# voidful/DeSTA2.5-Audio

Hardware: AMD Instinct MI355X
Metric: train steps/sec (node) Whisper-v3+Llama3.1-8B Q-Former6L at 1/2/4/8 MI355X (higher is better)
Workload: dtype bf16

## Files before the change

### desta2.5-audio_amd/csrc/attention.hip

```cpp
#include "common.h"
#include <mutex>
#include "desta_hip.h"

#ifndef ATTN_ABL
#define ATTN_ABL 0
#endif

namespace {

typedef __attribute__((ext_vector_type(4))) __bf16 bf16x4;

struct AttnArgs {
    const bf16_t* Q; const bf16_t* K; const bf16_t* V; bf16_t* O;
    const bf16_t* dO; bf16_t* dQ; bf16_t* dK; bf16_t* dV;
    float* lse; const float* delta;
    float* O32;
    const float* rope_cs;
    long q_bs, q_rs, k_bs, k_rs, v_bs, v_rs, o_bs, o_rs;
    long do_bs, do_rs, dq_bs, dq_rs, dk_bs, dk_rs, dv_bs, dv_rs;
    int B, Hq, Hkv, Sq, Sk;
    int causal;
    const int* kv_start;
    float scale_log2;
    float scale;
// ... 8 lines not shown
}

template <int N> struct stage_vec;
template <> struct stage_vec<1> { typedef __attribute__((ext_vector_type(4))) unsigned type; };
template <> struct stage_vec<2> { typedef __attribute__((ext_vector_type(8))) unsigned type; };
template <> struct stage_vec<4> { typedef __attribute__((ext_vector_type(16))) unsigned type; };
template <int D, int ROWS, int NT = 256> using stage_t = typename stage_vec<ROWS * (D / 8) / NT>::type;

template <int D, int ROWS, int NT = 256>
__device__ __forceinline__ stage_t<D, ROWS, NT> tile_load(const bf16_t* base, long rs, int row0, int max_row) {
    constexpr int CH = D / 8, N = ROWS * CH / NT;
    stage_t<D, ROWS, NT> out;
#pragma unroll
    for (int i = 0; i < N; ++i) {
        const int id = i * NT + threadIdx.x;
        const int r = id / CH, c = id % CH;
        const int gr = min(row0 + r, max_row);
        const uint4 v = *(const uint4*)(base + (long)gr * rs + c * 8);
        out[4 * i + 0] = v.x; out[4 * i + 1] = v.y; out[4 * i + 2] = v.z; out[4 * i + 3] = v.w;
    }
    return out;
}
template <int D, int ROWS, int NT = 256>
__device__ __forceinline__ void tile_store(char* img, const stage_t<D, ROWS, NT>& regs) {
    constexpr int CH = D / 8, N = ROWS * CH / NT;
#pragma unroll
    for (int i = 0; i < N; ++i) {
        const int id = i * NT + threadIdx.x;
        const int r = id / CH, c = id % CH;
        *(uint4*)(img + img_off<D>(r, c)) = make_uint4(regs[4 * i + 0], regs[4 * i + 1], regs[4 * i + 2], regs[4 * i + 3]);
    }
}

template <int D>
__device__ __forceinline__ bf16x8 frag_rows(const char* img, int row0, int ks, int lane) {
    const int r = row0 + (lane & 31);
    return *(const bf16x8*)(img + img_off<D>(r, 2 * ks + (lane >> 5)));
}

template <int D>
__device__ __forceinline__ bf16x8 frag_tr(const char* img, int row0, int col0, int lane) {
    const int i = lane & 15, g = (lane >> 4) & 1, h = lane >> 5;
    const int q = i >> 2, pp = i & 3;
    const int c = col0 + 16 * g + 4 * pp;
    const int r_lo = row0 + 4 * h + q;
    const int a0 = img_off<D>(r_lo, c >> 3) + ((c & 4) << 1);
    const int a1 = img_off<D>(r_lo + 8, c >> 3) + ((c & 4) << 1);
    const bf16x4 lo = __builtin_amdgcn_ds_read_tr16_b64_v4bf16((__attribute__((address_space(3))) bf16x4*)(img + a0));
    const bf16x4 hi = __builtin_amdgcn_ds_read_tr16_b64_v4bf16((__attribute__((address_space(3))) bf16x4*)(img + a1));
    bf16x8 out;
    out[0] = lo[0]; out[1] = lo[1]; out[2] = lo[2]; out[3] = lo[3];
    out[4] = hi[0]; out[5] = hi[1]; out[6] = hi[2]; out[7] = hi[3];
    return out;
}

__device__ __forceinline__ bf16x8 acc_frag(const f32x16& x, int s) {
    bf16x8 o;
#pragma unroll
    for (int j = 0; j < 8; ++j) o[j] = (__bf16)x[8 * s + j];
    return o;
}

__device__ __forceinline__ int acc_row(int reg, int lane) { return (reg & 3) + 8 * (reg >> 2) + 4 * (lane >> 5); }

__device__ __forceinline__ void attn_work_item(const AttnArgs& p, int nq, int& qblk, int& h, int& b) {
    const int id = blockIdx.x, per = nq * (p.Hq / p.Hkv), ngrp = p.B * p.Hkv;
    int g, r;
    if ((ngrp & 7) == 0) {
        const int xcd = id & 7, slot = id >> 3;
        g = (slot / per) * 8 + xcd;
        r = slot % per;
    } else {
        g = id / per;
        r = id % per;
    }
    b = g / p.Hkv;
    h = (g % p.Hkv) * (p.Hq / p.Hkv) + r / nq;
    qblk = r % nq;
    if (p.causal) qblk = nq - 1 - qblk;
}

#ifndef ATTN_FWD_PF
#define ATTN_FWD_PF 1
#endif
#ifndef ATTN_FWD64_WAVES
#define ATTN_FWD64_WAVES 3
#endif
template <int D, bool DROP, int NW = 4>
__global__ __launch_bounds__(64 * NW, NW == 4 ? (D == 64 ? ATTN_FWD64_WAVES : 2) : 2) void attn_fwd_k(AttnArgs p) {
    constexpr int NT = 64 * NW, QB = 32 * NW;
    __shared__ __attribute__((aligned(16))) char lds[2 * 64 * D * 2];
    char* kimg = lds;
    char* vimg = lds + 64 * D * 2;
    const int lane = threadIdx.x & 63, wave = __builtin_amdgcn_readfirstlane(threadIdx.x >> 6), h2 = lane >> 5;
    int qblk, h, b;
    attn_work_item(p, (p.Sq + QB - 1) / QB, qblk, h, b);
    const int qb0 = qblk * QB, q0 = qb0 + wave * 32;
    const int hk = h / (p.Hq / p.Hkv);
    const int qcol = q0 + (lane & 31);

    const bf16_t* qptr = p.Q + (long)b * p.q_bs + (long)min(qcol, p.Sq - 1) * p.q_rs + (long)h * D;
    bf16x8 qf[D / 16];
#pragma unroll
    for (int ds = 0; ds < D / 16; ++ds) qf[ds] = *(const bf16x8*)(qptr + 16 * ds + 8 * h2);

    const int coff = p.Sk - p.Sq;
    const int kv_lo = p.kv_start ? max(0, min(p.kv_start[b], p.Sk)) : 0;
    int kv_hi = p.Sk;
    if (p.causal) kv_hi = min(p.Sk, min(qb0 + QB - 1, p.Sq - 1) + coff + 1);
    const int t_lo = kv_lo / 64, t_hi = (kv_hi + 63) / 64;
    const int q_abs = qcol + coff;
    const int wave_kmax = p.causal ? min(q0 + 31, p.Sq - 1) + coff : p.Sk - 1;

    const bf16_t* kbase = p.K + (long)b * p.k_bs + (long)hk * D;
    const bf16_t* vbase = p.V + (long)b * p.v_bs + (long)hk * D;

    f32x16 oacc[D / 32];
#pragma unroll
    for (int i = 0; i < D / 32; ++i)
#pragma unroll
        for (int r = 0; r < 16; ++r) oacc[i][r] = 0.f;
    float m = -INFINITY, l = 0.f;

    constexpr int PF = ATTN_FWD_PF;
    stage_t<D, 64, NT> kr0 = {}, vr0 = {}, kr1 = {}, vr1 = {};
    if (t_lo < t_hi) {
        kr0 = tile_load<D, 64, NT>(kbase, p.k_rs, t_lo * 64, p.Sk - 1);
        vr0 = tile_load<D, 64, NT>(vbase, p.v_rs, t_lo * 64, p.Sk - 1);
    }
    if (PF == 2 && t_lo + 1 < t_hi) {
        kr1 = tile_load<D, 64, NT>(kbase, p.k_rs, (t_lo + 1) * 64, p.Sk - 1);
        vr1 = tile_load<D, 64, NT>(vbase, p.v_rs, (t_lo + 1) * 64, p.Sk - 1);
    }
    auto compute = [&](const int kt) __attribute__((always_inline)) {
        if (kt * 64 > wave_kmax) return;
        f32x16 st[2];
#pragma unroll
        for (int kb = 0; kb < 2; ++kb)
#pragma unroll
            for (int r = 0; r < 16; ++r) st[kb][r] = 0.f;
        {
            constexpr int NS = (ATTN_ABL == 4 ? 1 : D / 16);
            bf16x8 ka[NS], kbf[NS];
#pragma unroll
            for (int ds = 0; ds < NS; ++ds) ka[ds] = frag_rows<D>(kimg, 0, ds, lane);
            __builtin_amdgcn_sched_barrier(0);
#pragma unroll
            for (int ds = 0; ds < NS; ++ds) {
                st[0] = __builtin_amdgcn_mfma_f32_32x32x16_bf16(ka[ds], qf[ds], st[0], 0, 0, 0);
                kbf[ds] = frag_rows<D>(kimg, 32, ds, lane);
            }
            __builtin_amdgcn_sched_barrier(0);
#pragma unroll
            for (int ds = 0; ds < NS; ++ds) st[1] = __builtin_amdgcn_mfma_f32_32x32x16_bf16(kbf[ds], qf[ds], st[1], 0, 0, 0);
        }
        const bool need_mask = (kt * 64 + 63 >= p.Sk) || (kt * 64 < kv_lo) || (p.causal && kt * 64 + 63 > q0 + coff);
        if (need_mask) {
            asm volatile("; boundary tile" ::: "memory");
#pragma unroll
            for (int kb = 0; kb < 2; ++kb)
#pragma unroll
                for (int r = 0; r < 16; ++r) {
                    const int key = kt * 64 + kb * 32 + acc_row(r, lane);
                    const bool ok = key < p.Sk && key >= kv_lo && (!p.causal || key <= q_abs);
                    st[kb][r] = ok ? st[kb][r] : -INFINITY;
                }
        }
        float tmax = -INFINITY;
#pragma unroll
        for (int kb = 0; kb < 2; ++kb)
#pragma unroll
            for (int r = 0; r < 16; ++r) tmax = fmaxf(tmax, st[kb][r]);
        tmax = fmaxf(tmax, __shfl_xor(tmax, 32, 64)) * p.scale_log2;
        const float mnew = fmaxf(m, tmax);
        const float muse = (mnew == -INFINITY) ? 0.f : mnew;
        const float alpha = __builtin_amdgcn_exp2f(m - muse);
        typedef float f32x2 __attribute__((ext_vector_type(2)));
        f32x2 rs2 = {0.f, 0.f};
        const f32x2 sc2 = {p.scale_log2, p.scale_log2}, nm2 = {-muse, -muse};
#pragma unroll
        for (int kb = 0; kb < 2; ++kb)
#pragma unroll
            for (int r = 0; r < 16; r += 2) {
                const f32x2 sv = {st[kb][r], st[kb][r + 1]};
                const f32x2 av = sv * sc2 + nm2;
                f32x2 pv;
                pv.x = ATTN_ABL == 3 ? sv.x : __builtin_amdgcn_exp2f(av.x);
                pv.y = ATTN_ABL == 3 ? sv.y : __builtin_amdgcn_exp2f(av.y);
                st[kb][r] = pv.x;
                st[kb][r + 1] = pv.y;
                rs2 += pv;
            }
        float rs = rs2.x + rs2.y;
        rs += __shfl_xor(rs, 32, 64);
        l = l * alpha + rs;
        if constexpr (DROP) {
            const unsigned long rowbase = (((unsigned long)b * p.Hq + h) * p.Sq + min(qcol, p.Sq - 1)) * p.Sk;
#pragma unroll
            for (int kb = 0; kb < 2; ++kb)
#pragma unroll
                for (int r = 0; r < 16; r += 2) {
                    const unsigned long i0 = rowbase + (kt * 64 + kb * 32 + acc_row(r, lane));
                    const unsigned hsh = desta_rng32(p.seed_lo, p.seed_hi, i0 >> 1);
                    st[kb][r] = (hsh & 0xffffu) >= p.drop_thresh ? st[kb][r] * p.drop_scale : 0.f;
                    st[kb][r + 1] = (hsh >> 16) >= p.drop_thresh ? st[kb][r + 1] * p.drop_scale : 0.f;
                }
        }
        if (__any(mnew != m)) {
#pragma unroll
            for (int i = 0; i < D / 32; ++i)
#pragma unroll
                for (int r = 0; r < 16; ++r) oacc[i][r] *= alpha;
        }
        m = mnew;
#pragma unroll
        for (int kb = 0; kb < 2; ++kb)
#pragma unroll
            for (int s = 0; s < 2; ++s) {
                const bf16x8 pb = acc_frag(st[kb], s);
#pragma unroll
                for (int i = 0; i < (ATTN_ABL == 5 ? 1 : D / 32); ++i)
                    oacc[i] = __builtin_amdgcn_mfma_f32_32x32x16_bf16(frag_tr<D>(vimg, kb * 32 + 16 * s, i * 32, lane), pb, oacc[i], 0, 0, 0);
            }
    };
#define DESTA_KV_STAGE(KT, KR, VR)                                                   \
    __syncthreads();                         \
    asm volatile("; stage " #KR ::: "memory");  \
    if (ATTN_ABL != 1 || (KT) == t_lo) {                                             \
    tile_store<D, 64, NT>(kimg, KR);                                                     \
    tile_store<D, 64, NT>(vimg, VR);                                                     \
    }                                                                                \
    __syncthreads();                                                                 \
    if (ATTN_ABL != 2 && (KT) + PF < t_hi) {                                         \
        KR = tile_load<D, 64, NT>(kbase, p.k_rs, ((KT) + PF) * 64, p.Sk - 1);            \
        VR = tile_load<D, 64, NT>(vbase, p.v_rs, ((KT) + PF) * 64, p.Sk - 1);            \
    }
    for (int kt = t_lo; kt < t_hi; kt += 2) {
        DESTA_KV_STAGE(kt, kr0, vr0)
        compute(kt);
        if (kt + 1 < t_hi) {
            if constexpr (PF == 2) {
                DESTA_KV_STAGE(kt + 1, kr1, vr1)
            } else {
                DESTA_KV_STAGE(kt + 1, kr0, vr0)
            }
            compute(kt + 1);
        }
    }
#undef DESTA_KV_STAGE

    if (qcol < p.Sq) {
        const float inv = l > 0.f ? 1.0f / l : 0.f;
        bf16_t* optr = p.O + (long)b * p.o_bs + (long)qcol * p.o_rs + (long)h * D;
#pragma unroll
        for (int i = 0; i < D / 32; ++i)
#pragma unroll
            for (int rq = 0; rq < 4; ++rq) {
                u16x4 o;
#pragma unroll
                for (int e = 0; e < 4; ++e) o[e] = f2bf(oacc[i][4 * rq + e] * inv);
                *(u16x4*)(optr + i * 32 + 8 * rq + 4 * h2) = o;
            }
        if (p.O32) {
            float* o32 = p.O32 + (long)b * p.o_bs + (long)qcol * p.o_rs + (long)h * D;
#pragma unroll
            for (int i = 0; i < D / 32; ++i)
#pragma unroll
                for (int rq = 0; rq < 4; ++rq)
                    *(f32x4*)(o32 + i * 32 + 8 * rq + 4 * h2) = f32x4{oacc[i][4 * rq] * inv, oacc[i][4 * rq + 1] * inv, oacc[i][4 * rq + 2] * inv, oacc[i][4 * rq + 3] * inv};
        }
        if (p.lse && h2 == 0) p.lse[((long)b * p.Hq + h) * p.Sq + qcol] = l > 0.f ? m + log2f(l) : INFINITY;
    }
}

#ifndef ATTN_DEFER_LOG2
#define ATTN_DEFER_LOG2 6.0f
#endif
__device__ __forceinline__ float vmax3(float a, float b, float c) {
    float r;
    asm("v_max3_f32 %0, %1, %2, %3" : "=v"(r) : "v"(a), "v"(b), "v"(c));
    return r;
}
__device__ __forceinline__ float vmax2(float a, float b) {
    float r;
    asm("v_max_f32 %0, %1, %2" : "=v"(r) : "v"(a), "v"(b));
    return r;
}
__device__ __forceinline__ float swap_halves_max(float x) {
    const unsigned u = __builtin_bit_cast(unsigned, x);
    const auto r = __builtin_amdgcn_permlane32_swap(u, u, false, false);
    return vmax2(__builtin_bit_cast(float, (unsigned)r[0]), __builtin_bit_cast(float, (unsigned)r[1]));
}
__device__ __forceinline__ float swap_halves_sum(float x) {
    const unsigned u = __builtin_bit_cast(unsigned, x);
    const auto r = __builtin_amdgcn_permlane32_swap(u, u, false, false);
    return __builtin_bit_cast(float, (unsigned)r[0]) + __builtin_bit_cast(float, (unsigned)r[1]);
}
__device__ __forceinline__ bf16x8 tr_pair(const char* lo, const char* hi) {
    const bf16x4 a = __builtin_amdgcn_ds_read_tr16_b64_v4bf16((__attribute__((address_space(3))) bf16x4*)lo);
    const bf16x4 c = __builtin_amdgcn_ds_read_tr16_b64_v4bf16((__attribute__((address_space(3))) bf16x4*)hi);
    return __builtin_shufflevector(a, c, 0, 1, 2, 3, 4, 5, 6, 7);
}

template <int D, bool CAUSAL, int HPB, int MINW = 2, bool STAGGER = false>
__global__ __launch_bounds__(512, MINW) void attn_fwd8_k(AttnArgs p) {
    constexpr int NT = 512, RB = 256 / HPB, WPH = RB / 32;
    constexpr int TILE = 64 * D * 2;
    constexpr int SLOT = 2 * TILE, NSLOT = STAGGER ? 3 : 2;
    constexpr int NCH = 64 * (D / 8) / NT;
    __shared__ __attribute__((aligned(16))) char lds[NSLOT * SLOT];
    const int lane = threadIdx.x & 63, wave = __builtin_amdgcn_readfirstlane(threadIdx.x >> 6), h2 = lane >> 5;
    const int G = p.Hq / p.Hkv, nq = (p.Sq + RB - 1) / RB, hgroups = G / HPB, ngrp = p.B * p.Hkv;
    int g, qblk, hg;
    {
        const int id = blockIdx.x, per = nq * hgroups;
        if ((ngrp & 7) == 0) {
            const int xcd = id & 7, slot = id >> 3, gpx = ngrp >> 3;
            if (CAUSAL) {
                const int r = slot % (hgroups * gpx);
                qblk = nq - 1 - slot / (hgroups * gpx); hg = r / gpx; g = (r % gpx) * 8 + xcd;
            } else {
                const int r = slot % per;
                g = (slot / per) * 8 + xcd; hg = r / nq; qblk = r % nq;
            }
        } else if (CAUSAL) {
            const int r = id % (hgroups * ngrp);
            qblk = nq - 1 - id / (hgroups * ngrp); hg = r / ngrp; g = r % ngrp;
        } else {
            const int r = id % per;
            g = id / per; hg = r / nq; qblk = r % nq;
        }
    }
    const int b = g / p.Hkv, hk = g % p.Hkv;
    const int h = hk * G + hg * HPB + wave / WPH;
    const int qb0 = qblk * RB, q0 = qb0 + (wave % WPH) * 32;
    const int qcol = q0 + (lane & 31);
    const bool wave_on = q0 < p.Sq;

    const int coff = p.Sk - p.Sq;
    const int kv_lo = p.kv_start ? max(0, min(p.kv_start[b], p.Sk)) : 0;
    int kv_hi = p.Sk;
    if (CAUSAL) kv_hi = min(p.Sk, min(qb0 + RB - 1, p.Sq - 1) + coff + 1);
    const int t_lo = kv_lo / 64, t_hi = (kv_hi + 63) / 64;
    const int q_abs = qcol + coff;
    const int wave_kmax = CAUSAL ? min(q0 + 31, p.Sq - 1) + coff : p.Sk - 1;

    const char* kbase = (const char*)(p.K + (long)b * p.k_bs + (long)hk * D);
    const char* vbase = (const char*)(p.V + (long)b * p.v_bs + (long)hk * D);
    int srow[NCH], sdst[NCH];
    unsigned ksrc[NCH], vsrc[NCH];
#pragma unroll
    for (int i = 0; i < NCH; ++i) {
        const int id = i * NT + threadIdx.x, r = id / (D / 8), c = id % (D / 8);
        srow[i] = r;
        sdst[i] = img_off<D>(r, c);
        ksrc[i] = (unsigned)(r * (int)p.k_rs + c * 8) * 2u;
        vsrc[i] = (unsigned)(r * (int)p.v_rs + c * 8) * 2u;
    }
    typedef typename stage_vec<NCH>::type stage8_t;
    stage8_t kr = {}, vr = {};
    auto load_tile = [&](const int kt) __attribute__((always_inline)) {
        const char* kb_ = kbase + (long)kt * 64 * p.k_rs * 2;
        const char* vb_ = vbase + (long)kt * 64 * p.v_rs * 2;
        const bool ragged = kt * 64 + 64 > p.Sk;
#pragma unroll
        for (int i = 0; i < NCH; ++i) {
            unsigned ko = ksrc[i], vo = vsrc[i];
            if (ragged) {
                const int rc = max(min(srow[i], p.Sk - 1 - kt * 64), -kt * 64), c = (i * NT + (int)threadIdx.x) % (D / 8);
                ko = (unsigned)(rc * (int)p.k_rs + c * 8) * 2u;
                vo = (unsigned)(rc * (int)p.v_rs + c * 8) * 2u;
            }
            const uint4 a = *(const uint4*)(kb_ + (long)(int)ko), c4 = *(const uint4*)(vb_ + (long)(int)vo);
            kr[4 * i + 0] = a.x; kr[4 * i + 1] = a.y; kr[4 * i + 2] = a.z; kr[4 * i + 3] = a.w;
            vr[4 * i + 0] = c4.x; vr[4 * i + 1] = c4.y; vr[4 * i + 2] = c4.z; vr[4 * i + 3] = c4.w;
        }
    };
    auto store_tile = [&](char* slot) __attribute__((always_inline)) {
#pragma unroll
        for (int i = 0; i < NCH; ++i) {
            *(uint4*)(slot + sdst[i]) = make_uint4(kr[4 * i + 0], kr[4 * i + 1], kr[4 * i + 2], kr[4 * i + 3]);
            *(uint4*)(slot + TILE + sdst[i]) = make_uint4(vr[4 * i + 0], vr[4 * i + 1], vr[4 * i + 2], vr[4 * i + 3]);
        }
    };

    load_tile(t_lo);
    const bf16_t* qptr = p.Q + (long)b * p.q_bs + (long)min(qcol, p.Sq - 1) * p.q_rs + (long)h * D;
    bf16x8 qf[D / 16];
#pragma unroll
    for (int ds = 0; ds < D / 16; ++ds) qf[ds] = *(const bf16x8*)(qptr + 16 * ds + 8 * h2);
#pragma unroll
    for (int ds = 0; ds < D / 16; ++ds) asm volatile("" :: "v"(qf[ds]));
    store_tile(lds);
    load_tile(t_lo + 1);

    int kofs[D / 16], vofs[D / 32][2];
#pragma unroll
    for (int ds = 0; ds < D / 16; ++ds) {
        kofs[ds] = img_off<D>(lane & 31, 2 * ds + h2);
        asm volatile("" : "+v"(kofs[ds]));
    }
    {
        const int i16 = lane & 15, gq = (lane >> 4) & 1, qq = i16 >> 2, pp = i16 & 3;
#pragma unroll
        for (int i = 0; i < D / 32; ++i) {
            const int c = i * 32 + 16 * gq + 4 * pp;
            vofs[i][0] = TILE + img_off<D>(4 * h2 + qq, c >> 3) + ((c & 4) << 1);
            vofs[i][1] = TILE + img_off<D>(4 * h2 + qq + 8, c >> 3) + ((c & 4) << 1);
            asm volatile("" : "+v"(vofs[i][0]), "+v"(vofs[i][1]));
        }
    }

    f32x16 oacc[D / 32];
#pragma unroll
    for (int i = 0; i < D / 32; ++i)
#pragma unroll
        for (int r = 0; r < 16; ++r) oacc[i][r] = 0.f;
    float m = -INFINITY, l = 0.f;
    f32x16 st[2];
#define ATTN_BARRIER() asm volatile("s_waitcnt lgkmcnt(0)\n\ts_barrier" ::: "memory")
    ATTN_BARRIER();

    auto scores = [&](const int kt, const int sb) __attribute__((always_inline)) {
        if (!(wave_on && kt * 64 <= wave_kmax)) return;
#pragma unroll
        for (int kb = 0; kb < 2; ++kb)
#pragma unroll
            for (int r = 0; r < 16; ++r) st[kb][r] = 0.f;
        bf16x8 ka[D / 16], kbf[D / 16];
        int kad[D / 16];
#pragma unroll
        for (int ds = 0; ds < D / 16; ++ds) { kad[ds] = kofs[ds] + sb; asm volatile("" : "+v"(kad[ds])); }
#pragma unroll
        for (int ds = 0; ds < D / 16; ++ds) ka[ds] = *(const bf16x8*)(lds + kad[ds]);
        __builtin_amdgcn_sched_barrier(0);
#pragma unroll
        for (int ds = 0; ds < D / 16; ++ds) {
            st[0] = __builtin_amdgcn_mfma_f32_32x32x16_bf16(ka[ds], qf[ds], st[0], 0, 0, 0);
            kbf[ds] = *(const bf16x8*)(lds + kad[ds] + 32 * D * 2);
        }
        __builtin_amdgcn_sched_barrier(0);
#pragma unroll
        for (int ds = 0; ds < D / 16; ++ds) st[1] = __builtin_amdgcn_mfma_f32_32x32x16_bf16(kbf[ds], qf[ds], st[1], 0, 0, 0);
        const bool need_mask = (kt * 64 + 63 >= p.Sk) || (kt * 64 < kv_lo) || (CAUSAL && kt * 64 + 63 > q0 + coff);
        if (need_mask) {
            asm volatile("; boundary tile" ::: "memory");
#pragma unroll
            for (int kb = 0; kb < 2; ++kb)
#pragma unroll
                for (int r = 0; r < 16; ++r) {
                    const int key = kt * 64 + kb * 32 + acc_row(r, lane);
                    const bool ok = key < p.Sk && key >= kv_lo && (!CAUSAL || key <= q_abs);
                    st[kb][r] = ok ? st[kb][r] : -INFINITY;
                }
        }
        float tmax = vmax3(st[0][0], st[1][0], st[0][1]);
        tmax = vmax3(tmax, st[1][1], st[0][2]);
#pragma unroll
        for (int r = 2; r < 15; ++r) tmax = vmax3(tmax, st[1][r], st[0][r + 1]);
        tmax = vmax2(tmax, st[1][15]);
        tmax = swap_halves_max(tmax) * p.scale_log2;
        if (!__all(!(tmax > m + ATTN_DEFER_LOG2))) {
            const float mnew = vmax2(m, tmax);
            const float alpha = __builtin_amdgcn_exp2f(m - (mnew == -INFINITY ? 0.f : mnew));
            l *= alpha;
#pragma unroll
            for (int i = 0; i < D / 32; ++i)
#pragma unroll
                for (int r = 0; r < 16; ++r) oacc[i][r] *= alpha;
            m = mnew;
        }
        const float nmu = (m == -INFINITY) ? 0.f : -m;
#pragma unroll
        for (int kb = 0; kb < 2; ++kb)
#pragma unroll
            for (int r = 0; r < 16; ++r) {
                st[kb][r] = __builtin_amdgcn_exp2f(fmaf(st[kb][r], p.scale_log2, nmu));
                l += st[kb][r];
            }
    };
    auto pv = [&](const int kt, const int sb) __attribute__((always_inline)) {
        if (!(wave_on && kt * 64 <= wave_kmax)) return;
        int vad[D / 32][2];
#pragma unroll
        for (int i = 0; i < D / 32; ++i)
#pragma unroll
            for (int j = 0; j < 2; ++j) { vad[i][j] = vofs[i][j] + sb; asm volatile("" : "+v"(vad[i][j])); }
#pragma unroll
        for (int kb = 0; kb < 2; ++kb)
#pragma unroll
            for (int s = 0; s < 2; ++s) {
                const bf16x8 pb = acc_frag(st[kb], s);
#pragma unroll
                for (int i = 0; i < D / 32; ++i)
                    oacc[i] = __builtin_amdgcn_mfma_f32_32x32x16_bf16(
                        tr_pair(lds + vad[i][0] + (kb * 32 + 16 * s) * D * 2, lds + vad[i][1] + (kb * 32 + 16 * s) * D * 2), pb, oacc[i], 0, 0, 0);
            }
    };
    auto stage = [&](const int kt, const int sb_next) __attribute__((always_inline)) {
        if (kt + 1 < t_hi) {
            store_tile(lds + sb_next);
            if (kt + 2 < t_hi) load_tile(kt + 2);
        }
    };
    auto next_slot = [](int sb) { return sb == (NSLOT - 1) * SLOT ? 0 : sb + SLOT; };
    int sb = 0;
    if (!STAGGER || wave < 4) {
        for (int kt = t_lo; kt < t_hi; ++kt) {
            const int sn = next_slot(sb);
            scores(kt, sb);
            stage(kt, sn);
            pv(kt, sb);
            ATTN_BARRIER();
            sb = sn;
        }
    } else if (t_lo < t_hi) {
        scores(t_lo, sb);
        stage(t_lo, next_slot(sb));
        ATTN_BARRIER();
        for (int kt = t_lo; kt + 1 < t_hi; ++kt) {
            const int sn = next_slot(sb);
            pv(kt, sb);
            stage(kt + 1, next_slot(sn));
            scores(kt + 1, sn);
            ATTN_BARRIER();
            sb = sn;
        }
        pv(t_hi - 1, sb);
    }
#undef ATTN_BARRIER

    if (wave_on && qcol < p.Sq) {
        const float lt = swap_halves_sum(l);
        const float inv = lt > 0.f ? 1.0f / lt : 0.f;
        bf16_t* optr = p.O + (long)b * p.o_bs + (long)qcol * p.o_rs + (long)h * D;
#pragma unroll
        for (int i = 0; i < D / 32; ++i)
#pragma unroll
            for (int j = 0; j < 2; ++j) {
                unsigned a[2], c[2];
#pragma unroll
                for (int e = 0; e < 2; ++e) {
                    a[e] = (unsigned)f2bf(oacc[i][8 * j + 2 * e] * inv) | ((unsigned)f2bf(oacc[i][8 * j + 2 * e + 1] * inv) << 16);
                    c[e] = (unsigned)f2bf(oacc[i][8 * j + 4 + 2 * e] * inv) | ((unsigned)f2bf(oacc[i][8 * j + 4 + 2 * e + 1] * inv) << 16);
                }
                const auto r0 = __builtin_amdgcn_permlane32_swap(a[0], c[0], false, false);
                const auto r1 = __builtin_amdgcn_permlane32_swap(a[1], c[1], false, false);
                *(uint4*)(optr + i * 32 + 16 * j + 8 * h2) = make_uint4(r0[0], r1[0], r0[1], r1[1]);
            }
        if (p.O32) {
            float* o32 = p.O32 + (long)b * p.o_bs + (long)qcol * p.o_rs + (long)h * D;
#pragma unroll
            for (int i = 0; i < D / 32; ++i)
#pragma unroll
                for (int rq = 0; rq < 4; ++rq)
                    *(f32x4*)(o32 + i * 32 + 8 * rq + 4 * h2) = f32x4{oacc[i][4 * rq] * inv, oacc[i][4 * rq + 1] * inv, oacc[i][4 * rq + 2] * inv, oacc[i][4 * rq + 3] * inv};
        }
        if (p.lse && h2 == 0) p.lse[((long)b * p.Hq + h) * p.Sq + qcol] = lt > 0.f ? m + log2f(lt) : INFINITY;
    }
}

template <int D>
__global__ __launch_bounds__(256) void attn_delta_k(AttnArgs p, float* __restrict__ delta) {
    constexpr int G = D / 8;
    const long gid = (long)blockIdx.x * 256 + threadIdx.x;
    const long rowid = gid / G;
    const int j = (int)(gid % G);
    const long total = (long)p.B * p.Hq * p.Sq;
    const bool active = rowid < total;
    const long rr = active ? rowid : 0;
    const int q = (int)(rr % p.Sq), h = (int)((rr / p.Sq) % p.Hq), b = (int)(rr / ((long)p.Sq * p.Hq));
    const u16x8 g = *(const u16x8*)(p.dO + (long)b * p.do_bs + (long)q * p.do_rs + (long)h * D + 8 * j);
    float s = 0.f;
    if (p.O32) {
        const float* o32 = p.O32 + (long)b * p.o_bs + (long)q * p.o_rs + (long)h * D + 8 * j;
        const f32x4 o0 = *(const f32x4*)o32, o1 = *(const f32x4*)(o32 + 4);
#pragma unroll
        for (int e = 0; e < 4; ++e) s += o0[e] * bf2f(g[e]) + o1[e] * bf2f(g[4 + e]);
    } else {
        const u16x8 o = *(const u16x8*)(p.O + (long)b * p.o_bs + (long)q * p.o_rs + (long)h * D + 8 * j);
#pragma unroll
        for (int e = 0; e < 8; ++e) s += bf2f(o[e]) * bf2f(g[e]);
    }
#pragma unroll
    for (int o2 = 1; o2 < G; o2 <<= 1) s += __shfl_xor(s, o2, 64);
    if (active && j == 0) delta[rowid] = s;
}

#ifndef ATTN_DQ_PF
#define ATTN_DQ_PF 1
#endif
#ifndef ATTN_DQ_BLOCKS
#define ATTN_DQ_BLOCKS 2
#endif
template <int D, bool DROP, int NW = 4>
__global__ __launch_bounds__(64 * NW, NW == 4 ? ATTN_DQ_BLOCKS : 2) void attn_bwd_dq_k(AttnArgs p) {
    constexpr int NT = 64 * NW, QB = 32 * NW;
    __shared__ __attribute__((aligned(16))) char lds[2 * 64 * D * 2];
    char* kimg = lds;
    char* vimg = lds + 64 * D * 2;
    const int lane = threadIdx.x & 63, wave = __builtin_amdgcn_readfirstlane(threadIdx.x >> 6), h2 = lane >> 5;
    int qblk, h, b;
    attn_work_item(p, (p.Sq + QB - 1) / QB, qblk, h, b);
    const int qb0 = qblk * QB, q0 = qb0 + wave * 32;
    const int hk = h / (p.Hq / p.Hkv);
    const int qcol = q0 + (lane & 31), qc = min(qcol, p.Sq - 1);

    const bf16_t* qptr = p.Q + (long)b * p.q_bs + (long)qc * p.q_rs + (long)h * D;
    const bf16_t* gptr = p.dO + (long)b * p.do_bs + (long)qc * p.do_rs + (long)h * D;
    bf16x8 qf[D / 16], gf[D / 16];
#pragma unroll
    for (int ds = 0; ds < D / 16; ++ds) {
        qf[ds] = *(const bf16x8*)(qptr + 16 * ds + 8 * h2);
        gf[ds] = *(const bf16x8*)(gptr + 16 * ds + 8 * h2);
    }
    const long stat = ((long)b * p.Hq + h) * p.Sq + qc;
    const float lse = p.lse[stat], dlt = p.delta[stat];

    const int coff = p.Sk - p.Sq;
    const int kv_lo = p.kv_start ? max(0, min(p.kv_start[b], p.Sk)) : 0;
    int kv_hi = p.Sk;
    if (p.causal) kv_hi = min(p.Sk, min(qb0 + QB - 1, p.Sq - 1) + coff + 1);
    const int t_lo = kv_lo / 64, t_hi = (kv_hi + 63) / 64;
    const int q_abs = qcol + coff;
    const int wave_kmax = p.causal ? min(q0 + 31, p.Sq - 1) + coff : p.Sk - 1;

    const bf16_t* kbase = p.K + (long)b * p.k_bs + (long)hk * D;
    const bf16_t* vbase = p.V + (long)b * p.v_bs + (long)hk * D;

    f32x16 dq[D / 32];
#pragma unroll
    for (int i = 0; i < D / 32; ++i)
#pragma unroll
        for (int r = 0; r < 16; ++r) dq[i][r] = 0.f;

    constexpr int PF = ATTN_DQ_PF;
    stage_t<D, 64, NT> kr0 = {}, vr0 = {}, kr1 = {}, vr1 = {};
    if (t_lo < t_hi) {
        kr0 = tile_load<D, 64, NT>(kbase, p.k_rs, t_lo * 64, p.Sk - 1);
        vr0 = tile_load<D, 64, NT>(vbase, p.v_rs, t_lo * 64, p.Sk - 1);
    }
    if (PF == 2 && t_lo + 1 < t_hi) {
        kr1 = tile_load<D, 64, NT>(kbase, p.k_rs, (t_lo + 1) * 64, p.Sk - 1);
        vr1 = tile_load<D, 64, NT>(vbase, p.v_rs, (t_lo + 1) * 64, p.Sk - 1);
    }
    auto compute = [&](const int kt) __attribute__((always_inline)) {
        if (kt * 64 > wave_kmax) return;
#pragma unroll
        for (int kb = 0; kb < 2; ++kb) {
            f32x16 st, dp;
#pragma unroll
            for (int r = 0; r < 16; ++r) { st[r] = 0.f; dp[r] = 0.f; }
#pragma unroll
            for (int ds = 0; ds < D / 16; ++ds) {
                st = __builtin_amdgcn_mfma_f32_32x32x16_bf16(frag_rows<D>(kimg, kb * 32, ds, lane), qf[ds], st, 0, 0, 0);
                dp = __builtin_amdgcn_mfma_f32_32x32x16_bf16(frag_rows<D>(vimg, kb * 32, ds, lane), gf[ds], dp, 0, 0, 0);
            }
            const bool need_mask = (kt * 64 + kb * 32 + 31 >= p.Sk) || (kt * 64 + kb * 32 < kv_lo) ||
                                   (p.causal && kt * 64 + kb * 32 + 31 > q0 + coff);
            unsigned keep = 0xffffu;
            if constexpr (DROP) {
                const unsigned long rowbase = (((unsigned long)b * p.Hq + h) * p.Sq + qc) * p.Sk;
                keep = 0;
#pragma unroll
                for (int r = 0; r < 16; r += 2) {
                    const unsigned long i0 = rowbase + (kt * 64 + kb * 32 + acc_row(r, lane));
                    const unsigned hsh = desta_rng32(p.seed_lo, p.seed_hi, i0 >> 1);
                    keep |= ((hsh & 0xffffu) >= p.drop_thresh ? 1u : 0u) << r;
                    keep |= ((hsh >> 16) >= p.drop_thresh ? 1u : 0u) << (r + 1);
                }
            }
            if (need_mask) {
                asm volatile("; boundary tile" ::: "memory");
#pragma unroll
                for (int r = 0; r < 16; ++r) {
                    const int key = kt * 64 + kb * 32 + acc_row(r, lane);
                    const bool ok = key < p.Sk && key >= kv_lo && (!p.causal || key <= q_abs);
                    st[r] = ok ? st[r] : -INFINITY;
                }
            }
#pragma unroll
            for (int r = 0; r < 16; ++r) {
                const float pv = __builtin_amdgcn_exp2f(fmaf(st[r], p.scale_log2, -lse));
                float dpr = dp[r];
                if constexpr (DROP) dpr = ((keep >> r) & 1u) ? dpr * p.drop_scale : 0.f;
                st[r] = pv * (dpr - dlt) * p.scale;
            }
#pragma unroll
            for (int s = 0; s < 2; ++s) {
                const bf16x8 dsf = acc_frag(st, s);
#pragma unroll
                for (int i = 0; i < D / 32; ++i)
                    dq[i] = __builtin_amdgcn_mfma_f32_32x32x16_bf16(frag_tr<D>(kimg, kb * 32 + 16 * s, i * 32, lane), dsf, dq[i], 0, 0, 0);
            }
        }
    };
#define DESTA_KV_STAGE(KT, KR, VR)                                                   \
    __syncthreads();                         \
    asm volatile("; stage " #KR ::: "memory");  \
    tile_store<D, 64, NT>(kimg, KR);                                                     \
    tile_store<D, 64, NT>(vimg, VR);                                                     \
    __syncthreads();                                                                 \
    if ((KT) + PF < t_hi) {                                                          \
        KR = tile_load<D, 64, NT>(kbase, p.k_rs, ((KT) + PF) * 64, p.Sk - 1);            \
        VR = tile_load<D, 64, NT>(vbase, p.v_rs, ((KT) + PF) * 64, p.Sk - 1);            \
    }
    for (int kt = t_lo; kt < t_hi; kt += 2) {
        DESTA_KV_STAGE(kt, kr0, vr0)
        compute(kt);
        if (kt + 1 < t_hi) {
            if constexpr (PF == 2) {
                DESTA_KV_STAGE(kt + 1, kr1, vr1)
            } else {
                DESTA_KV_STAGE(kt + 1, kr0, vr0)
            }
            compute(kt + 1);
        }
    }
#undef DESTA_KV_STAGE
    if (qcol < p.Sq) {
        bf16_t* optr = p.dQ + (long)b * p.dq_bs + (long)qcol * p.dq_rs + (long)h * D;
#pragma unroll
        for (int i = 0; i < D / 32; ++i)
#pragma unroll
            for (int rq = 0; rq < 4; ++rq) {
                u16x4 o;
#pragma unroll
                for (int e = 0; e < 4; ++e) o[e] = f2bf(dq[i][4 * rq + e]);
                *(u16x4*)(optr + i * 32 + 8 * rq + 4 * h2) = o;
            }
    }
}

template <int D, bool CAUSAL, int HPB>
__global__ __launch_bounds__(512, 2) void attn_bwd_dq8_k(AttnArgs p, float* __restrict__ delta_out) {
    constexpr int NT = 512, RB = 256 / HPB, WPH = RB / 32;
    constexpr int TILE = 64 * D * 2, SLOT = 2 * TILE;
    constexpr int NCH = 64 * (D / 8) / NT;
    __shared__ __attribute__((aligned(16))) char lds[2 * SLOT];
    const int lane = threadIdx.x & 63, wave = __builtin_amdgcn_readfirstlane(threadIdx.x >> 6), h2 = lane >> 5;
    const int G = p.Hq / p.Hkv, nq = (p.Sq + RB - 1) / RB, hgroups = G / HPB, ngrp = p.B * p.Hkv;
    int g, qblk, hg;
    {
        const int id = blockIdx.x, per = nq * hgroups;
        if ((ngrp & 7) == 0) {
            const int xcd = id & 7, slot = id >> 3, gpx = ngrp >> 3;
            if (CAUSAL) {
                const int r = slot % (hgroups * gpx);
                qblk = nq - 1 - slot / (hgroups * gpx); hg = r / gpx; g = (r % gpx) * 8 + xcd;
            } else {
                const int r = slot % per;
                g = (slot / per) * 8 + xcd; hg = r / nq; qblk = r % nq;
            }
        } else if (CAUSAL) {
            const int r = id % (hgroups * ngrp);
            qblk = nq - 1 - id / (hgroups * ngrp); hg = r / ngrp; g = r % ngrp;
        } else {
            const int r = id % per;
            g = id / per; hg = r / nq; qblk = r % nq;
        }
    }
    const int b = g / p.Hkv, hk = g % p.Hkv;
    const int h = hk * G + hg * HPB + wave / WPH;
    const int qb0 = qblk * RB, q0 = qb0 + (wave % WPH) * 32;
    const int qcol = q0 + (lane & 31), qc = min(qcol, p.Sq - 1);
    const bool wave_on = q0 < p.Sq;

    const int coff = p.Sk - p.Sq;
    const int kv_lo = p.kv_start ? max(0, min(p.kv_start[b], p.Sk)) : 0;
    int kv_hi = p.Sk;
    if (CAUSAL) kv_hi = min(p.Sk, min(qb0 + RB - 1, p.Sq - 1) + coff + 1);
    const int t_lo = kv_lo / 64, t_hi = (kv_hi + 63) / 64;
    const int q_abs = qcol + coff;
    const int wave_kmax = CAUSAL ? min(q0 + 31, p.Sq - 1) + coff : p.Sk - 1;

    const char* kbase = (const char*)(p.K + (long)b * p.k_bs + (long)hk * D);
    const char* vbase = (const char*)(p.V + (long)b * p.v_bs + (long)hk * D);
    int srow[NCH], sdst[NCH];
    unsigned ksrc[NCH], vsrc[NCH];
#pragma unroll
    for (int i = 0; i < NCH; ++i) {
        const int id = i * NT + threadIdx.x, r = id / (D / 8), c = id % (D / 8);
        srow[i] = r;
        sdst[i] = img_off<D>(r, c);
        ksrc[i] = (unsigned)(r * (int)p.k_rs + c * 8) * 2u;
        vsrc[i] = (unsigned)(r * (int)p.v_rs + c * 8) * 2u;
    }
    typedef typename stage_vec<NCH>::type stage8_t;
    stage8_t kr = {}, vr = {};
    auto load_tile = [&](const int kt) __attribute__((always_inline)) {
        const char* kb_ = kbase + (long)kt * 64 * p.k_rs * 2;
        const char* vb_ = vbase + (long)kt * 64 * p.v_rs * 2;
        const bool ragged = kt * 64 + 64 > p.Sk;
#pragma unroll
        for (int i = 0; i < NCH; ++i) {
            unsigned ko = ksrc[i], vo = vsrc[i];
            if (ragged) {
                const int rc = max(min(srow[i], p.Sk - 1 - kt * 64), -kt * 64), c = (i * NT + (int)threadIdx.x) % (D / 8);
                ko = (unsigned)(rc * (int)p.k_rs + c * 8) * 2u;
                vo = (unsigned)(rc * (int)p.v_rs + c * 8) * 2u;
            }
            const uint4 a = *(const uint4*)(kb_ + (long)(int)ko), c4 = *(const uint4*)(vb_ + (long)(int)vo);
            kr[4 * i + 0] = a.x; kr[4 * i + 1] = a.y; kr[4 * i + 2] = a.z; kr[4 * i + 3] = a.w;
            vr[4 * i + 0] = c4.x; vr[4 * i + 1] = c4.y; vr[4 * i + 2] = c4.z; vr[4 * i + 3] = c4.w;
        }
    };
    auto store_tile = [&](char* slot) __attribute__((always_inline)) {
#pragma unroll
        for (int i = 0; i < NCH; ++i) {
            *(uint4*)(slot + sdst[i]) = make_uint4(kr[4 * i + 0], kr[4 * i + 1], kr[4 * i + 2], kr[4 * i + 3]);
            *(uint4*)(slot + TILE + sdst[i]) = make_uint4(vr[4 * i + 0], vr[4 * i + 1], vr[4 * i + 2], vr[4 * i + 3]);
        }
    };

    load_tile(t_lo);
    const bf16_t* qptr = p.Q + (long)b * p.q_bs + (long)qc * p.q_rs + (long)h * D;
    const bf16_t* gptr = p.dO + (long)b * p.do_bs + (long)qc * p.do_rs + (long)h * D;
    const bf16_t* optr = p.O + (long)b * p.o_bs + (long)qc * p.o_rs + (long)h * D;
    bf16x8 qf[D / 16], gf[D / 16];
    float dl = 0.f;
#pragma unroll
    for (int ds = 0; ds < D / 16; ++ds) {
        qf[ds] = *(const bf16x8*)(qptr + 16 * ds + 8 * h2);
        gf[ds] = *(const bf16x8*)(gptr + 16 * ds + 8 * h2);
        const bf16x8 of = *(const bf16x8*)(optr + 16 * ds + 8 * h2);
#pragma unroll
        for (int j = 0; j < 8; ++j) dl += (float)of[j] * (float)gf[ds][j];
    }
    const long stat = ((long)b * p.Hq + h) * p.Sq + qc;
    const float nlse = -p.lse[stat];
    const float dlt = swap_halves_sum(dl);
    if (wave_on && qcol < p.Sq && h2 == 0) delta_out[stat] = dlt;
#pragma unroll
    for (int ds = 0; ds < D / 16; ++ds) asm volatile("" :: "v"(qf[ds]), "v"(gf[ds]));
    asm volatile("" :: "v"(nlse));
    store_tile(lds);
    load_tile(t_lo + 1);

    int kofs[D / 16], tofs[D / 32][2];
#pragma unroll
    for (int ds = 0; ds < D / 16; ++ds) {
        kofs[ds] = img_off<D>(lane & 31, 2 * ds + h2);
        asm volatile("" : "+v"(kofs[ds]));
    }
    {
        const int i16 = lane & 15, gq = (lane >> 4) & 1, qq = i16 >> 2, pp = i16 & 3;
#pragma unroll
        for (int i = 0; i < D / 32; ++i) {
            const int c = i * 32 + 16 * gq + 4 * pp;
            tofs[i][0] = img_off<D>(4 * h2 + qq, c >> 3) + ((c & 4) << 1);
            tofs[i][1] = img_off<D>(4 * h2 + qq + 8, c >> 3) + ((c & 4) << 1);
            asm volatile("" : "+v"(tofs[i][0]), "+v"(tofs[i][1]));
        }
    }
    f32x16 dq[D / 32];
#pragma unroll
    for (int i = 0; i < D / 32; ++i)
#pragma unroll
        for (int r = 0; r < 16; ++r) dq[i][r] = 0.f;
#define ATTN_BARRIER() asm volatile("s_waitcnt lgkmcnt(0)\n\ts_barrier" ::: "memory")
    ATTN_BARRIER();

    int sb = 0;
    for (int kt = t_lo; kt < t_hi; ++kt) {
        const int sn = SLOT - sb;
        const bool act = wave_on && kt * 64 <= wave_kmax;
        if (act) {
            int kad[D / 16];
#pragma unroll
            for (int ds = 0; ds < D / 16; ++ds) { kad[ds] = kofs[ds] + sb; asm volatile("" : "+v"(kad[ds])); }
#pragma unroll
            for (int kb = 0; kb < 2; ++kb) {
                if (CAUSAL && kt * 64 + kb * 32 > wave_kmax) break;
                f32x16 st, dp;
#pragma unroll
                for (int r = 0; r < 16; ++r) { st[r] = 0.f; dp[r] = 0.f; }
#pragma unroll
                for (int ds = 0; ds < D / 16; ++ds) {
                    st = __builtin_amdgcn_mfma_f32_32x32x16_bf16(*(const bf16x8*)(lds + kad[ds] + kb * 32 * D * 2), qf[ds], st, 0, 0, 0);
                    dp = __builtin_amdgcn_mfma_f32_32x32x16_bf16(*(const bf16x8*)(lds + kad[ds] + TILE + kb * 32 * D * 2), gf[ds], dp, 0, 0, 0);
                }
                const bool need_mask = (kt * 64 + kb * 32 + 31 >= p.Sk) || (kt * 64 + kb * 32 < kv_lo) ||
                                       (CAUSAL && kt * 64 + kb * 32 + 31 > q0 + coff);
                if (need_mask) {
                    asm volatile("; boundary tile" ::: "memory");
#pragma unroll
                    for (int r = 0; r < 16; ++r) {
                        const int key = kt * 64 + kb * 32 + acc_row(r, lane);
                        const bool ok = key < p.Sk && key >= kv_lo && (!CAUSAL || key <= q_abs);
                        st[r] = ok ? st[r] : -INFINITY;
                    }
                }
#pragma unroll
                for (int r = 0; r < 16; ++r) {
                    const float pv = __builtin_amdgcn_exp2f(fmaf(st[r], p.scale_log2, nlse));
                    st[r] = pv * ((dp[r] - dlt) * p.scale);
                }
                int tad[D / 32][2];
#pragma unroll
                for (int i = 0; i < D / 32; ++i)
#pragma unroll
                    for (int j = 0; j < 2; ++j) { tad[i][j] = tofs[i][j] + sb + kb * 32 * D * 2; asm volatile("" : "+v"(tad[i][j])); }
#pragma unroll
                for (int s = 0; s < 2; ++s) {
                    const bf16x8 dsf = acc_frag(st, s);
#pragma unroll
                    for (int i = 0; i < D / 32; ++i)
                        dq[i] = __builtin_amdgcn_mfma_f32_32x32x16_bf16(tr_pair(lds + tad[i][0] + 16 * s * D * 2, lds + tad[i][1] + 16 * s * D * 2), dsf, dq[i], 0, 0, 0);
                }
            }
        }
        if (kt + 1 < t_hi) {
            store_tile(lds + sn);
            if (kt + 2 < t_hi) load_tile(kt + 2);
        }
        ATTN_BARRIER();
        sb = sn;
    }
#undef ATTN_BARRIER

    if (wave_on && qcol < p.Sq) {
        bf16_t* dqp = p.dQ + (long)b * p.dq_bs + (long)qcol * p.dq_rs + (long)h * D;
        if (p.rope_cs) {
            const float* cs = p.rope_cs + (long)qcol * D;
#pragma unroll
            for (int i = 0; i < D / 32; ++i)
#pragma unroll
                for (int jj = 0; jj < 4; ++jj) {
                    const float4 c4 = *(const float4*)(cs + (32 * i + 8 * jj + 4 * h2));
                    const float g0 = dq[i][4 * jj], g1 = dq[i][4 * jj + 1], g2 = dq[i][4 * jj + 2], g3 = dq[i][4 * jj + 3];
                    dq[i][4 * jj] = g0 * c4.x + g1 * c4.y;     dq[i][4 * jj + 1] = g1 * c4.x - g0 * c4.y;
                    dq[i][4 * jj + 2] = g2 * c4.z + g3 * c4.w; dq[i][4 * jj + 3] = g3 * c4.z - g2 * c4.w;
                }
        }
#pragma unroll
        for (int i = 0; i < D / 32; ++i)
#pragma unroll
            for (int j = 0; j < 2; ++j) {
                unsigned a[2], c[2];
#pragma unroll
                for (int e = 0; e < 2; ++e) {
                    a[e] = (unsigned)f2bf(dq[i][8 * j + 2 * e]) | ((unsigned)f2bf(dq[i][8 * j + 2 * e + 1]) << 16);
                    c[e] = (unsigned)f2bf(dq[i][8 * j + 4 + 2 * e]) | ((unsigned)f2bf(dq[i][8 * j + 4 + 2 * e + 1]) << 16);
                }
                const auto r0 = __builtin_amdgcn_permlane32_swap(a[0], c[0], false, false);
                const auto r1 = __builtin_amdgcn_permlane32_swap(a[1], c[1], false, false);
                *(uint4*)(dqp + i * 32 + 16 * j + 8 * h2) = make_uint4(r0[0], r1[0], r0[1], r1[1]);
            }
    }
}

#ifndef ATTN_DKDV_QR
#define ATTN_DKDV_QR 32
#endif

template <int D, bool DROP, int NW = 4>
__global__ __launch_bounds__(64 * NW, (NW == 4 && D == 64) ? 2 : 1) void attn_bwd_dkdv_k(AttnArgs p) {
    constexpr int QR = (D == 128) ? ATTN_DKDV_QR : 32;
    constexpr int NT = 64 * NW, KB = 32 * NW;
    constexpr int LDS_LOOP = 2 * QR * D * 2 + 2 * QR * 4, LDS_EPI = NW * 32 * 64 * 4;
    __shared__ __attribute__((aligned(16))) char lds[LDS_LOOP > LDS_EPI ? LDS_LOOP : LDS_EPI];
    char* qimg = lds;
    char* gimg = lds + QR * D * 2;
    float* lse_s = (float*)(lds + 2 * QR * D * 2);
    float* dlt_s = lse_s + QR;
    const int lane = threadIdx.x & 63, wave = __builtin_amdgcn_readfirstlane(threadIdx.x >> 6), h2 = lane >> 5;
    const int nhb = p.Hkv * p.B;
    const int kb0 = (blockIdx.x / nhb) * KB, k0 = kb0 + wave * 32;
    const int hk = (blockIdx.x % nhb) % p.Hkv, b = (blockIdx.x % nhb) / p.Hkv, group = p.Hq / p.Hkv;
    const int kcol = k0 + (lane & 31), kc = min(kcol, p.Sk - 1);
    const int kv_lo = p.kv_start ? max(0, min(p.kv_start[b], p.Sk)) : 0;
    const int coff = p.Sk - p.Sq;

    const bf16_t* kptr = p.K + (long)b * p.k_bs + (long)kc * p.k_rs + (long)hk * D;
    const bf16_t* vptr = p.V + (long)b * p.v_bs + (long)kc * p.v_rs + (long)hk * D;
    bf16x8 kf[D / 16], vf[D / 16];
#pragma unroll
    for (int ds = 0; ds < D / 16; ++ds) {
        kf[ds] = *(const bf16x8*)(kptr + 16 * ds + 8 * h2);
        vf[ds] = *(const bf16x8*)(vptr + 16 * ds + 8 * h2);
    }
    const bool key_ok = kcol < p.Sk && kcol >= kv_lo;

    f32x16 dk[D / 32], dv[D / 32];
#pragma unroll
    for (int i = 0; i < D / 32; ++i)
#pragma unroll
        for (int r = 0; r < 16; ++r) { dk[i][r] = 0.f; dv[i][r] = 0.f; }

    const int q_first = p.causal ? max(0, kb0 - coff) : 0;
    const int qt_lo = q_first / QR, qt_hi = (p.Sq + QR - 1) / QR;
    const int nq = qt_hi - qt_lo, n_it = group * nq;
    stage_t<D, QR, NT> qr0 = {}, gr0 = {}, qr1 = {}, gr1 = {};
    float ls0 = 0.f, dl0 = 0.f, ls1 = 0.f, dl1 = 0.f;
#define DESTA_Q_FETCH(IT, QR_, GR, LS, DL)                                                                      \
    {                                                                                                          \
        const int h_ = hk * group + (IT) / nq, qt_ = qt_lo + (IT) % nq;                                        \
        QR_ = tile_load<D, QR, NT>(p.Q + (long)b * p.q_bs + (long)h_ * D, p.q_rs, qt_ * QR, p.Sq - 1);        \
        GR = tile_load<D, QR, NT>(p.dO + (long)b * p.do_bs + (long)h_ * D, p.do_rs, qt_ * QR, p.Sq - 1);      \
        if (threadIdx.x < QR) {                                                                                \
            const long st_ = ((long)b * p.Hq + h_) * p.Sq + min(qt_ * QR + (int)threadIdx.x, p.Sq - 1);       \
            LS = p.lse[st_];                                                                                   \
            DL = p.delta[st_];                                                                                 \
        }                                                                                                      \
    }
#define DESTA_Q_STAGE(IT, QR_, GR, LS, DL)                                                                      \
    __syncthreads();                                                                                           \
    asm volatile("; stage " #QR_ ::: "memory");                                                                \
    tile_store<D, QR, NT>(qimg, QR_);                                                                          \
    tile_store<D, QR, NT>(gimg, GR);                                                                           \
    if (threadIdx.x < QR) { lse_s[threadIdx.x] = LS; dlt_s[threadIdx.x] = DL; }                                \
    __syncthreads();                                                                                           \
    if ((IT) + 2 < n_it) DESTA_Q_FETCH((IT) + 2, QR_, GR, LS, DL)
    if (n_it > 0) DESTA_Q_FETCH(0, qr0, gr0, ls0, dl0)
    if (n_it > 1) DESTA_Q_FETCH(1, qr1, gr1, ls1, dl1)
    auto compute = [&](const int it) __attribute__((always_inline)) {
        const int qt = qt_lo + it % nq;
        constexpr int NS = QR / 32;
        f32x16 stv[NS], dpv[NS];
        bool act[NS];
#pragma unroll
        for (int sub = 0; sub < NS; ++sub) {
            const int qb = qt * QR + sub * 32;
            act[sub] = qb < p.Sq && !(p.causal && k0 > qb + 31 + coff);
            if (!act[sub]) continue;
#pragma unroll
            for (int r = 0; r < 16; ++r) { stv[sub][r] = 0.f; dpv[sub][r] = 0.f; }
#pragma unroll
            for (int ds = 0; ds < D / 16; ++ds) {
                stv[sub] = __builtin_amdgcn_mfma_f32_32x32x16_bf16(frag_rows<D>(qimg, sub * 32, ds, lane), kf[ds], stv[sub], 0, 0, 0);
                dpv[sub] = __builtin_amdgcn_mfma_f32_32x32x16_bf16(frag_rows<D>(gimg, sub * 32, ds, lane), vf[ds], dpv[sub], 0, 0, 0);
            }
        }
#pragma unroll
        for (int sub = 0; sub < NS; ++sub) {
            if (!act[sub]) continue;
            const int qb = qt * QR + sub * 32;
            f32x16& st = stv[sub];
            f32x16& dp = dpv[sub];
            const bool need_mask = (qb + 31 >= p.Sq) || (k0 + 31 >= p.Sk) || (k0 < kv_lo) ||
                                   (p.causal && k0 + 31 > qb + coff);
            float lsv[16], dlv[16];
#pragma unroll
            for (int q4 = 0; q4 < 4; ++q4) {
                const float4 a4 = *(const float4*)(lse_s + sub * 32 + 8 * q4 + 4 * h2);
                const float4 b4 = *(const float4*)(dlt_s + sub * 32 + 8 * q4 + 4 * h2);
                lsv[4 * q4 + 0] = a4.x; lsv[4 * q4 + 1] = a4.y; lsv[4 * q4 + 2] = a4.z; lsv[4 * q4 + 3] = a4.w;
                dlv[4 * q4 + 0] = b4.x; dlv[4 * q4 + 1] = b4.y; dlv[4 * q4 + 2] = b4.z; dlv[4 * q4 + 3] = b4.w;
            }
            unsigned keep = 0xffffu;
            if constexpr (DROP) {
                const unsigned long hb = ((unsigned long)b * p.Hq + (hk * group + it / nq)) * p.Sq;
                keep = 0;
                const int half = lane & 1, kpair = k0 + (lane & 30);
                unsigned hh[8];
#pragma unroll
                for (int j = 0; j < 8; ++j) {
                    const int ql = (j & 3) + 8 * (2 * half + (j >> 2)) + 4 * h2;
                    hh[j] = desta_rng32(p.seed_lo, p.seed_hi, ((hb + min(qb + ql, p.Sq - 1)) * p.Sk + kpair) >> 1);
                }
#pragma unroll
                for (int j = 0; j < 8; ++j) {
                    const unsigned oth = (unsigned)__builtin_amdgcn_mov_dpp((int)hh[j], 0xB1, 0xf, 0xf, true);
                    const unsigned mine = half ? (hh[j] >> 16) : (hh[j] & 0xffffu), theirs = half ? (oth >> 16) : (oth & 0xffffu);
                    keep |= (mine >= p.drop_thresh ? 1u : 0u) << (8 * half + j);
                    keep |= (theirs >= p.drop_thresh ? 1u : 0u) << (8 * (1 - half) + j);
                }
            }
            if (need_mask) {
                asm volatile("; boundary slice" ::: "memory");
#pragma unroll
                for (int r = 0; r < 16; ++r) {
                    const int q = qb + acc_row(r, lane);
                    const bool ok = key_ok && q < p.Sq && (!p.causal || kcol <= q + coff);
                    st[r] = ok ? st[r] : -INFINITY;
                }
            }
#pragma unroll
            for (int r = 0; r < 16; ++r) {
                const float pv = __builtin_amdgcn_exp2f(fmaf(st[r], p.scale_log2, -lsv[r]));
                float ms = 1.0f;
                if constexpr (DROP) ms = ((keep >> r) & 1u) ? p.drop_scale : 0.f;
                st[r] = pv * ms;
                dp[r] = pv * (ms * dp[r] - dlv[r]) * p.scale;
            }
#pragma unroll
            for (int s = 0; s < 2; ++s) {
                const bf16x8 pf = acc_frag(st, s), dsf = acc_frag(dp, s);
#pragma unroll
                for (int i = 0; i < D / 32; ++i) {
                    dv[i] = __builtin_amdgcn_mfma_f32_32x32x16_bf16(pf, frag_tr<D>(gimg, sub * 32 + 16 * s, i * 32, lane), dv[i], 0, 0, 0);
                    dk[i] = __builtin_amdgcn_mfma_f32_32x32x16_bf16(dsf, frag_tr<D>(qimg, sub * 32 + 16 * s, i * 32, lane), dk[i], 0, 0, 0);
                }
            }
        }
    };
    for (int it = 0; it < n_it; it += 2) {
        DESTA_Q_STAGE(it, qr0, gr0, ls0, dl0)
        compute(it);
        if (it + 1 < n_it) {
            DESTA_Q_STAGE(it + 1, qr1, gr1, ls1, dl1)
            compute(it + 1);
        }
    }
#undef DESTA_Q_STAGE
#undef DESTA_Q_FETCH
    bf16_t* dkp = p.dK + (long)b * p.dk_bs + (long)hk * D;
    bf16_t* dvp = p.dV + (long)b * p.dv_bs + (long)hk * D;
    const bool wide = ((p.dk_rs | p.dv_rs | p.dk_bs | p.dv_bs) & 7) == 0 && (((size_t)p.dK | (size_t)p.dV) & 15) == 0;
    if (wide) {
        __syncthreads();
        float* tb = (float*)lds + wave * (32 * 64);
        auto emit = [&](const f32x16 (&acc)[D / 32], bf16_t* base, long rs, const bool rope) __attribute__((always_inline)) {
#pragma unroll
            for (int hf = 0; hf < D / 64; ++hf) {
#pragma unroll
                for (int ii = 0; ii < 2; ++ii)
#pragma unroll
                    for (int r = 0; r < 16; ++r) tb[acc_row(r, lane) * 64 + ii * 32 + (lane & 31)] = acc[hf * 2 + ii][r];
                asm volatile("s_waitcnt lgkmcnt(0)" ::: "memory");
#pragma unroll
                for (int j = 0; j < 4; ++j) {
                    const int row = (lane >> 3) + 8 * j, key = k0 + row;
                    float4 x0 = *(const float4*)(tb + row * 64 + (lane & 7) * 8), x1 = *(const float4*)(tb + row * 64 + (lane & 7) * 8 + 4);
                    if (rope) {
                        const float* cs = p.rope_cs + (long)min(key, p.Sk - 1) * D + hf * 64 + (lane & 7) * 8;
                        const float4 c0 = *(const float4*)cs, c1 = *(const float4*)(cs + 4);
                        const float4 y0 = make_float4(x0.x * c0.x + x0.y * c0.y, x0.y * c0.x - x0.x * c0.y, x0.z * c0.z + x0.w * c0.w, x0.w * c0.z - x0.z * c0.w);
                        const float4 y1 = make_float4(x1.x * c1.x + x1.y * c1.y, x1.y * c1.x - x1.x * c1.y, x1.z * c1.z + x1.w * c1.w, x1.w * c1.z - x1.z * c1.w);
                        x0 = y0; x1 = y1;
                    }
                    u16x8 o;
                    o[0] = f2bf(x0.x); o[1] = f2bf(x0.y); o[2] = f2bf(x0.z); o[3] = f2bf(x0.w);
                    o[4] = f2bf(x1.x); o[5] = f2bf(x1.y); o[6] = f2bf(x1.z); o[7] = f2bf(x1.w);
                    if (key < p.Sk) *(u16x8*)(base + (long)key * rs + hf * 64 + (lane & 7) * 8) = o;
                }
                asm volatile("s_waitcnt lgkmcnt(0)" ::: "memory");
            }
        };
        emit(dk, dkp, p.dk_rs, p.rope_cs != nullptr);
        emit(dv, dvp, p.dv_rs, false);
        return;
    }
#pragma unroll
    for (int i = 0; i < D / 32; ++i)
#pragma unroll
        for (int r = 0; r < 16; ++r) {
            const int key = k0 + acc_row(r, lane);
            if (key < p.Sk) {
                dkp[(long)key * p.dk_rs + i * 32 + (lane & 31)] = f2bf(dk[i][r]);
                dvp[(long)key * p.dv_rs + i * 32 + (lane & 31)] = f2bf(dv[i][r]);
            }
        }
}

template <bool DROP, bool TR>
__global__ __launch_bounds__(256, 2) void attn_bwd_q64_k(AttnArgs p, float* __restrict__ dq_part, float* __restrict__ bias_part, int blocks_per_chunk) {
    constexpr int D = 64, WREG = 12288;
    __shared__ __attribute__((aligned(16))) char lds[2 * 64 * D * 2 + 4 * WREG + 2 * 64 * 4];
    char* qimg = lds;
    char* gimg = lds + 64 * D * 2;
    char* wreg = lds + 2 * 64 * D * 2;
    float* lse_s = (float*)(wreg + 4 * WREG);
    float* dlt_s = lse_s + 64;
    const int lane = threadIdx.x & 63, wave = __builtin_amdgcn_readfirstlane(threadIdx.x >> 6), h2 = lane >> 5;
    const int nbh = p.B * p.Hq;
    const int chunk = blockIdx.x / nbh, bh = blockIdx.x % nbh, b = bh / p.Hq, h = bh % p.Hq;
    const int nkb = (p.Sk + 127) / 128;
    const int kb_lo = chunk * blocks_per_chunk, kb_hi = min(kb_lo + blocks_per_chunk, nkb);
    const int kv_lo = p.kv_start ? max(0, min(p.kv_start[b], p.Sk)) : 0;
    char* kimg_w = wreg + wave * WREG;
    char* vimg_w = kimg_w + 4096;
    char* dsimg_w = kimg_w + 8192;
    const bf16_t* kbase = p.K + (long)b * p.k_bs + (long)h * D;
    const bf16_t* vbase = p.V + (long)b * p.v_bs + (long)h * D;

    {
        const stage_t<D, 64> qr = tile_load<D, 64>(p.Q + (long)b * p.q_bs + (long)h * D, p.q_rs, 0, p.Sq - 1);
        const stage_t<D, 64> gr = tile_load<D, 64>(p.dO + (long)b * p.do_bs + (long)h * D, p.do_rs, 0, p.Sq - 1);
        tile_store<D, 64>(qimg, qr);
        tile_store<D, 64>(gimg, gr);
        if (threadIdx.x < 64) {
            const long st_ = ((long)b * p.Hq + h) * p.Sq + min((int)threadIdx.x, p.Sq - 1);
            lse_s[threadIdx.x] = p.lse[st_];
            dlt_s[threadIdx.x] = p.delta[st_];
        }
    }
    const int qa = wave >> 1, di = wave & 1;
    f32x16 dq;
#pragma unroll
    for (int r = 0; r < 16; ++r) dq[r] = 0.f;

    stage_t<D, 128> kst = {}, vst = {};
    if (kb_lo < kb_hi) {
        kst = tile_load<D, 128>(kbase, p.k_rs, kb_lo * 128, p.Sk - 1);
        vst = tile_load<D, 128>(vbase, p.v_rs, kb_lo * 128, p.Sk - 1);
    }
    const unsigned long hb = ((unsigned long)b * p.Hq + h) * p.Sq;
    bf16_t* dkp = TR ? p.dK + (long)h * D * p.dkv_t_ld + (long)b * p.Sk : p.dK + (long)b * p.dk_bs + (long)h * D;
    bf16_t* dvp = TR ? p.dV + (long)h * D * p.dkv_t_ld + (long)b * p.Sk : p.dV + (long)b * p.dv_bs + (long)h * D;
    float bsum[2][2] = {{0.f, 0.f}, {0.f, 0.f}};

    for (int kb = kb_lo; kb < kb_hi; ++kb) {
        __syncthreads();
#pragma unroll
        for (int i = 0; i < 4; ++i) {
            const int id = i * 256 + threadIdx.x, r = id >> 3, c = id & 7;
            char* dst = wreg + (r >> 5) * WREG + img_off<D>(r & 31, c);
            *(uint4*)dst = make_uint4(kst[4 * i + 0], kst[4 * i + 1], kst[4 * i + 2], kst[4 * i + 3]);
            *(uint4*)(dst + 4096) = make_uint4(vst[4 * i + 0], vst[4 * i + 1], vst[4 * i + 2], vst[4 * i + 3]);
        }
        __syncthreads();
        if (kb + 1 < kb_hi) {
            kst = tile_load<D, 128>(kbase, p.k_rs, (kb + 1) * 128, p.Sk - 1);
            vst = tile_load<D, 128>(vbase, p.v_rs, (kb + 1) * 128, p.Sk - 1);
        }
        const int k0 = kb * 128 + wave * 32, kcol = k0 + (lane & 31);
        const bool key_ok = kcol < p.Sk && kcol >= kv_lo;
        f32x16 dk[2], dv[2];
#pragma unroll
        for (int i = 0; i < 2; ++i)
#pragma unroll
            for (int r = 0; r < 16; ++r) { dk[i][r] = 0.f; dv[i][r] = 0.f; }
#pragma unroll 1
        for (int sub = 0; sub < 2; ++sub) {
            const int qb = sub * 32;
            if (qb >= p.Sq) {
#pragma unroll
                for (int j = 0; j < 4; ++j) *(uint2*)(dsimg_w + img_off<D>(lane & 31, sub * 4 + j) + 8 * h2) = make_uint2(0u, 0u);
                continue;
            }
            unsigned keep = 0xffffu;
            if constexpr (DROP) {
                keep = 0;
                const int half = lane & 1, kpair = k0 + (lane & 30);
                unsigned hh[8];
                const unsigned long e0 = (hb + qb) * p.Sk + kpair;
#pragma unroll
                for (int j = 0; j < 8; ++j) {
                    const int ql = (j & 3) + 8 * (2 * half + (j >> 2)) + 4 * h2;
                    hh[j] = desta_rng32(p.seed_lo, p.seed_hi, (e0 + (unsigned)(ql * p.Sk)) >> 1);
                }
#pragma unroll
                for (int j = 0; j < 8; ++j) {
                    const unsigned oth = (unsigned)__builtin_amdgcn_mov_dpp((int)hh[j], 0xB1, 0xf, 0xf, true);
                    const unsigned mine = half ? (hh[j] >> 16) : (hh[j] & 0xffffu), theirs = half ? (oth >> 16) : (oth & 0xffffu);
                    keep |= (mine >= p.drop_thresh ? 1u : 0u) << (8 * half + j);
                    keep |= (theirs >= p.drop_thresh ? 1u : 0u) << (8 * (1 - half) + j);
                }
            }
            if constexpr (DROP) asm volatile("" : "+v"(keep));
            f32x16 st, dp;
// ... 306 lines not shown
        for (int j = 0; j < 8; ++j) {
            if constexpr (GP >= 4) {
                const float keep = hi16 ? a1[g + G2][j] : a1[g][j], send = hi16 ? a1[g][j] : a1[g + G2][j];
                a2[g][j] = keep + __shfl_xor(send, 16, 64);
            } else {
                a2[g][j] = a1[g][j] + __shfl_xor(a1[g][j], 16, 64);
            }
        }
    {
        const int gbase = (GP >= 2 && hi32 ? G1 : 0) + (GP >= 4 && hi16 ? G2 : 0);
        const bool writer = GP >= 4 ? true : (GP == 2 ? !hi16 : lane < 16);
        if (writer)
#pragma unroll
            for (int g = 0; g < G2; ++g) {
                float* dst = &s_red[wave][gbase + g][8 * c16];
                *(f32x4*)dst = f32x4{a2[g][0], a2[g][1], a2[g][2], a2[g][3]};
                *(f32x4*)(dst + 4) = f32x4{a2[g][4], a2[g][5], a2[g][6], a2[g][7]};
            }
    }
    __syncthreads();

    const int tg = threadIdx.x >> 5, d4 = threadIdx.x & 31;
    if (tg < G) {
        f32x4 o = *(const f32x4*)&s_red[0][tg][4 * d4];
#pragma unroll
        for (int w = 1; w < 4; ++w) o += *(const f32x4*)&s_red[w][tg][4 * d4];
        const float m = fmaxf(fmaxf(s_m[0][tg], s_m[1][tg]), fmaxf(s_m[2][tg], s_m[3][tg]));
        const float l = ((s_l[0][tg] + s_l[1][tg]) + s_l[2][tg]) + s_l[3][tg];
        const int h = hk * G + tg;
        if (nch == 1) {
            u16x4 ob;
#pragma unroll
            for (int e = 0; e < 4; ++e) ob[e] = f2bf(l > 0.f ? o[e] / l : 0.f);
            *(u16x4*)(p.O + (long)b * p.o_bs + (long)h * 128 + 4 * d4) = ob;
            if (p.lse && d4 == 0) p.lse[(long)b * p.Hq + h] = l > 0.f ? m + log2f(l) : INFINITY;
        } else {
            const long r = ((long)b * p.Hq + h) * nch + c;
            *(f32x4*)(ws_o + r * 128 + 4 * d4) = o;
            if (d4 == 0) { ws_ml[2 * r] = m; ws_ml[2 * r + 1] = l; }
        }
    }
}

__global__ __launch_bounds__(256) void attn_decode_combine_k(AttnArgs p, const float* __restrict__ ws_ml, const float* __restrict__ ws_o, int nch) {
    const long bh = (long)blockIdx.x * 8 + (threadIdx.x >> 5);
    const int d4 = threadIdx.x & 31;
    if (bh >= (long)p.B * p.Hq) return;
    const float* ml = ws_ml + 2 * bh * nch;
    const float* po = ws_o + bh * nch * 128 + 4 * d4;
    float m = -INFINITY;
    for (int c = 0; c < nch; ++c) m = fmaxf(m, ml[2 * c]);
    f32x4 o = {0.f, 0.f, 0.f, 0.f};
    float l = 0.f;
    for (int c = 0; c < nch; ++c) {
        const float mc = ml[2 * c], lc = ml[2 * c + 1];
        if (mc == -INFINITY || !(lc > 0.f)) continue;
        const float w = __builtin_amdgcn_exp2f(mc - m);
        const f32x4 oc = *(const f32x4*)(po + (long)c * 128);
        l = fmaf(w, lc, l);
#pragma unroll
        for (int e = 0; e < 4; ++e) o[e] = fmaf(w, oc[e], o[e]);
    }
    const int b = (int)(bh / p.Hq), h = (int)(bh % p.Hq);
    u16x4 ob;
#pragma unroll
    for (int e = 0; e < 4; ++e) ob[e] = f2bf(l > 0.f ? o[e] / l : 0.f);
    *(u16x4*)(p.O + (long)b * p.o_bs + (long)h * 128 + 4 * d4) = ob;
    if (p.lse && d4 == 0) p.lse[bh] = l > 0.f ? m + log2f(l) : INFINITY;
}

typedef __attribute__((ext_vector_type(2))) float f32x2;
__device__ __forceinline__ bf16x8 e4m3x8_to_bf16(const uint2& q) {
    union { unsigned u[4]; bf16x8 v; } o;
    const unsigned w[2] = {q.x, q.y};
#pragma unroll
    for (int i = 0; i < 2; ++i) {
        const f32x2 a = __builtin_amdgcn_cvt_pk_f32_fp8((int)w[i], false), b = __builtin_amdgcn_cvt_pk_f32_fp8((int)w[i], true);
        o.u[2 * i] = __builtin_amdgcn_perm(__float_as_uint(a[1]), __float_as_uint(a[0]), 0x07060302u);
        o.u[2 * i + 1] = __builtin_amdgcn_perm(__float_as_uint(b[1]), __float_as_uint(b[0]), 0x07060302u);
    }
    return o.v;
}
template <int GP>
__global__ __launch_bounds__(256) void attn_kv8_k(AttnArgs p, const float* __restrict__ k_scale, const float* __restrict__ v_scale, long sc_bs, long sc_rs,
                                                  float* __restrict__ ws_ml, float* __restrict__ ws_o, int nch) {
    constexpr int CH = DESTA_ATTN_DECODE_CHUNK, KW = CH / 4, NT16 = KW / 16, NV = KW / 4;
    __shared__ __attribute__((aligned(16))) float s_p[4][KW][8];
    __shared__ __attribute__((aligned(16))) float s_red[4][GP][128];
    __shared__ float s_m[4][8], s_l[4][8];
    const int lane = threadIdx.x & 63, wave = __builtin_amdgcn_readfirstlane(threadIdx.x >> 6), c16 = lane & 15, q4 = lane >> 4;
    const int G = p.Hq / p.Hkv;
    int id = blockIdx.x;
    const int c = id % nch; id /= nch;
    const int hk = id % p.Hkv, b = id / p.Hkv;
    const int kv_lo = p.kv_start ? max(0, min(p.kv_start[b], p.Sk)) : 0;
    const int k0 = c * CH + wave * KW;
    const bool live = k0 < p.Sk && k0 + KW > kv_lo;
    const int row_lo = min(kv_lo, p.Sk - 1), row_hi = p.Sk - 1;

    uint2 kq[NT16][4], vq[NV];
    float ksc[NT16][4], vsc[NT16][4];
    bf16x8 qf[4];
    if (live) {
        const uint8_t* kbase = (const uint8_t*)p.K + (long)b * p.k_bs + (long)hk * 128 + 8 * q4;
        const uint8_t* vbase = (const uint8_t*)p.V + (long)b * p.v_bs + (long)hk * 128 + 8 * c16;
        const float* ksb = k_scale + (long)b * sc_bs + hk;
        const float* vsb = v_scale + (long)b * sc_bs + hk;
#pragma unroll
        for (int t = 0; t < NT16; ++t) {
            const int row = min(max(k0 + 16 * t + c16, row_lo), row_hi);
#pragma unroll
            for (int ks = 0; ks < 4; ++ks) kq[t][ks] = *(const uint2*)(kbase + (long)row * p.k_rs + 32 * ks);
        }
#pragma unroll
        for (int i = 0; i < NV; ++i) {
            const int row = min(max(k0 + 4 * i + q4, row_lo), row_hi);
            vq[i] = *(const uint2*)(vbase + (long)row * p.v_rs);
        }
#pragma unroll
        for (int t = 0; t < NT16; ++t)
#pragma unroll
            for (int r = 0; r < 4; ++r) {
                const int row = min(max(k0 + 16 * t + 4 * q4 + r, row_lo), row_hi);
                ksc[t][r] = ksb[(long)row * sc_rs];
                vsc[t][r] = vsb[(long)row * sc_rs];
            }
    } else {
#pragma unroll
        for (int t = 0; t < NT16; ++t)
#pragma unroll
            for (int ks = 0; ks < 4; ++ks) { kq[t][ks] = make_uint2(0u, 0u); ksc[t][ks] = 1.f; vsc[t][ks] = 1.f; }
#pragma unroll
        for (int i = 0; i < NV; ++i) vq[i] = make_uint2(0u, 0u);
    }
    {
        const bf16_t* qptr = p.Q + (long)b * p.q_bs + (long)(hk * G + min(c16, G - 1)) * 128 + 8 * q4;
#pragma unroll
        for (int ks = 0; ks < 4; ++ks) {
            qf[ks] = *(const bf16x8*)(qptr + 32 * ks);
            if (c16 >= G)
#pragma unroll
                for (int j = 0; j < 8; ++j) qf[ks][j] = (__bf16)0.f;
        }
    }

    f32x4 st[NT16];
    float mx = -INFINITY;
#pragma unroll
    for (int t = 0; t < NT16; ++t) {
        st[t] = f32x4{0.f, 0.f, 0.f, 0.f};
#pragma unroll
        for (int ks = 0; ks < 4; ++ks) st[t] = __builtin_amdgcn_mfma_f32_16x16x32_bf16(e4m3x8_to_bf16(kq[t][ks]), qf[ks], st[t], 0, 0, 0);
#pragma unroll
        for (int r = 0; r < 4; ++r) {
            const int key = k0 + 16 * t + 4 * q4 + r;
            st[t][r] = (key >= kv_lo && key < p.Sk) ? (st[t][r] * ksc[t][r]) * p.scale_log2 : -INFINITY;
            mx = fmaxf(mx, st[t][r]);
        }
    }
    mx = fmaxf(mx, __shfl_xor(mx, 16, 64));
    mx = fmaxf(mx, __shfl_xor(mx, 32, 64));
    if (lane < 8) s_m[wave][lane] = mx;
    __syncthreads();
    const int g8 = c16 & 7;
    const float mblk = fmaxf(fmaxf(s_m[0][g8], s_m[1][g8]), fmaxf(s_m[2][g8], s_m[3][g8]));
    const float muse = (mblk == -INFINITY) ? 0.f : mblk;
    float ls = 0.f;
#pragma unroll
    for (int t = 0; t < NT16; ++t)
#pragma unroll
        for (int r = 0; r < 4; ++r) {
            const float pv = __builtin_amdgcn_exp2f(st[t][r] - muse);
            ls += pv;
            if (c16 < 8) s_p[wave][16 * t + 4 * q4 + r][c16] = pv * vsc[t][r];
        }
    ls += __shfl_xor(ls, 16, 64);
    ls += __shfl_xor(ls, 32, 64);
    if (lane < 8) s_l[wave][lane] = ls;
    __syncthreads();

    float acc[GP][8];
#pragma unroll
    for (int g = 0; g < GP; ++g)
#pragma unroll
        for (int j = 0; j < 8; ++j) acc[g][j] = 0.f;
#pragma unroll
    for (int i = 0; i < NV; ++i) {
        const float* pr = &s_p[wave][4 * i + q4][0];
        float pg[GP];
        if constexpr (GP >= 4) {
#pragma unroll
            for (int g = 0; g < GP; g += 4) {
                const f32x4 t4 = *(const f32x4*)(pr + g);
                pg[g] = t4[0]; pg[g + 1] = t4[1]; pg[g + 2] = t4[2]; pg[g + 3] = t4[3];
            }
        } else {
#pragma unroll
            for (int g = 0; g < GP; ++g) pg[g] = pr[g];
        }
        const f32x2 vv[4] = {__builtin_amdgcn_cvt_pk_f32_fp8((int)vq[i].x, false), __builtin_amdgcn_cvt_pk_f32_fp8((int)vq[i].x, true),
                             __builtin_amdgcn_cvt_pk_f32_fp8((int)vq[i].y, false), __builtin_amdgcn_cvt_pk_f32_fp8((int)vq[i].y, true)};
#pragma unroll
        for (int j2 = 0; j2 < 4; ++j2) {
            const float v0 = vv[j2][0], v1 = vv[j2][1];
#pragma unroll
            for (int g = 0; g < GP; ++g) {
                acc[g][2 * j2] = fmaf(pg[g], v0, acc[g][2 * j2]);
                acc[g][2 * j2 + 1] = fmaf(pg[g], v1, acc[g][2 * j2 + 1]);
            }
        }
    }
    const bool hi32 = (lane & 32) != 0, hi16 = (lane & 16) != 0;
    constexpr int G1 = GP >= 2 ? GP / 2 : GP, G2 = GP >= 4 ? GP / 4 : G1;
    float a1[G1][8], a2[G2][8];
#pragma unroll
    for (int g = 0; g < G1; ++g)
#pragma unroll
        for (int j = 0; j < 8; ++j) {
            if constexpr (GP >= 2) {
                const float keep = hi32 ? acc[g + G1][j] : acc[g][j], send = hi32 ? acc[g][j] : acc[g + G1][j];
                a1[g][j] = keep + __shfl_xor(send, 32, 64);
            } else {
                a1[g][j] = acc[g][j] + __shfl_xor(acc[g][j], 32, 64);
            }
        }
#pragma unroll
    for (int g = 0; g < G2; ++g)
#pragma unroll
        for (int j = 0; j < 8; ++j) {
            if constexpr (GP >= 4) {
                const float keep = hi16 ? a1[g + G2][j] : a1[g][j], send = hi16 ? a1[g][j] : a1[g + G2][j];
                a2[g][j] = keep + __shfl_xor(send, 16, 64);
            } else {
                a2[g][j] = a1[g][j] + __shfl_xor(a1[g][j], 16, 64);
            }
        }
    {
        const int gbase = (GP >= 2 && hi32 ? G1 : 0) + (GP >= 4 && hi16 ? G2 : 0);
        const bool writer = GP >= 4 ? true : (GP == 2 ? !hi16 : lane < 16);
        if (writer)
#pragma unroll
            for (int g = 0; g < G2; ++g) {
                float* dst = &s_red[wave][gbase + g][8 * c16];
                *(f32x4*)dst = f32x4{a2[g][0], a2[g][1], a2[g][2], a2[g][3]};
                *(f32x4*)(dst + 4) = f32x4{a2[g][4], a2[g][5], a2[g][6], a2[g][7]};
            }
    }
    __syncthreads();

    const int tg = threadIdx.x >> 5, d4 = threadIdx.x & 31;
    if (tg < G) {
        f32x4 o = *(const f32x4*)&s_red[0][tg][4 * d4];
#pragma unroll
        for (int w = 1; w < 4; ++w) o += *(const f32x4*)&s_red[w][tg][4 * d4];
        const float m = fmaxf(fmaxf(s_m[0][tg], s_m[1][tg]), fmaxf(s_m[2][tg], s_m[3][tg]));
        const float l = ((s_l[0][tg] + s_l[1][tg]) + s_l[2][tg]) + s_l[3][tg];
        const int h = hk * G + tg;
        if (nch == 1) {
            u16x4 ob;
#pragma unroll
            for (int e = 0; e < 4; ++e) ob[e] = f2bf(l > 0.f ? o[e] / l : 0.f);
            *(u16x4*)(p.O + (long)b * p.o_bs + (long)h * 128 + 4 * d4) = ob;
            if (p.lse && d4 == 0) p.lse[(long)b * p.Hq + h] = l > 0.f ? m + log2f(l) : INFINITY;
        } else {
            const long r = ((long)b * p.Hq + h) * nch + c;
            *(f32x4*)(ws_o + r * 128 + 4 * d4) = o;
            if (d4 == 0) { ws_ml[2 * r] = m; ws_ml[2 * r + 1] = l; }
        }
    }
}

int fill_args(const desta_attn_desc* d, AttnArgs& a) {
    DESTA_CHECK_ARG(d && d->Q && d->K && d->V, "attention: null operand");
    DESTA_CHECK_ARG(d->head_dim == 64 || d->head_dim == 128, "attention: head_dim %d unsupported (64 or 128)", d->head_dim);
    DESTA_CHECK_ARG(d->batch > 0 && d->n_q_heads > 0 && d->n_kv_heads > 0 && d->n_q_heads % d->n_kv_heads == 0,
                    "attention: bad head counts");
    DESTA_CHECK_ARG(d->seq_q > 0 && d->seq_k > 0, "attention: bad sequence lengths");
    DESTA_CHECK_ARG(!d->causal || d->seq_k >= d->seq_q, "attention: causal needs seq_k >= seq_q");
    DESTA_CHECK_ARG(d->q_row_stride % 8 == 0 && d->k_row_stride % 8 == 0 && d->v_row_stride % 8 == 0,
                    "attention: row strides must be multiples of 8 elements");
    DESTA_CHECK_ARG(d->batch <= 65535 && d->n_q_heads <= 65535, "attention: grid too large");
    a.Q = (const bf16_t*)d->Q; a.K = (const bf16_t*)d->K; a.V = (const bf16_t*)d->V; a.O = (bf16_t*)d->O;
    a.dO = (const bf16_t*)d->dO; a.dQ = (bf16_t*)d->dQ; a.dK = (bf16_t*)d->dK; a.dV = (bf16_t*)d->dV;
    a.lse = d->lse; a.delta = nullptr; a.O32 = d->O_f32; a.rope_cs = d->rope_cos_sin;
    a.q_bs = d->q_batch_stride; a.q_rs = d->q_row_stride; a.k_bs = d->k_batch_stride; a.k_rs = d->k_row_stride;
    a.v_bs = d->v_batch_stride; a.v_rs = d->v_row_stride; a.o_bs = d->o_batch_stride; a.o_rs = d->o_row_stride;
    a.do_bs = d->do_batch_stride; a.do_rs = d->do_row_stride; a.dq_bs = d->dq_batch_stride; a.dq_rs = d->dq_row_stride;
    a.dk_bs = d->dk_batch_stride; a.dk_rs = d->dk_row_stride; a.dv_bs = d->dv_batch_stride; a.dv_rs = d->dv_row_stride;
    a.B = d->batch; a.Hq = d->n_q_heads; a.Hkv = d->n_kv_heads; a.Sq = d->seq_q; a.Sk = d->seq_k;
    a.causal = d->causal; a.kv_start = d->kv_start;
    a.scale = d->scale; a.scale_log2 = d->scale * 1.44269504088896340736f;
    DESTA_CHECK_ARG(d->dropout_p >= 0.f && d->dropout_p < 1.f, "attention: dropout_p must be in [0,1)");
    DESTA_CHECK_ARG(d->dropout_p == 0.f || d->head_dim == 64, "attention: dropout is built for head_dim 64 (the Q-Former) only");
    DESTA_CHECK_ARG(d->dropout_p == 0.f || d->seq_k % 2 == 0, "attention: dropout needs an even seq_k (adjacent keys share one hash)");
    a.drop_thresh = d->dropout_p > 0.f ? desta_drop_thresh(d->dropout_p) : 0u;
    a.drop_scale = 1.0f / (1.0f - d->dropout_p);
    a.seed_lo = (unsigned)d->dropout_seed; a.seed_hi = (unsigned)(d->dropout_seed >> 32);
    a.dkv_t_ld = d->dkv_transposed ? d->dkv_t_ld : 0;
    return DESTA_OK;
}

}

namespace { int g_attn_opt[8] = {1, 0, 0, 0, 1, 0, 0, 0}; }
extern "C" int desta_attention_set_option(int which, int value) {
    DESTA_CHECK_ARG(which >= 0 && which < 8, "attention_set_option: unknown option %d", which);
    g_attn_opt[which] = value;
    return DESTA_OK;
}

extern "C" int desta_attention_fwd(const desta_attn_desc* d, void* stream) {
    AttnArgs a;
    if (int rc = fill_args(d, a)) return rc;
    DESTA_CHECK_ARG(d->O, "attention_fwd: null output");
    DESTA_CHECK_ARG(d->o_row_stride % 8 == 0 && d->o_batch_stride % 8 == 0 && ((size_t)d->O & 15) == 0,
                    "attention_fwd: O must be 16-byte aligned with row / batch strides that are multiples of 8 elements");
    if (g_attn_opt[0] && !a.drop_thresh && a.Sq >= 128) {
        const int G = a.Hq / a.Hkv;
        const int hpb = !a.causal ? 1 : (d->head_dim == 128 ? (G % 4 == 0 ? 4 : (G % 2 == 0 ? 2 : 1)) : (G % 2 == 0 ? 2 : 1));
        const int rb = 256 / hpb;
        dim3 g8((unsigned)((a.Sq + rb - 1) / rb) * (unsigned)(G / hpb) * (unsigned)(a.B * a.Hkv));
        hipStream_t st = (hipStream_t)stream;
        if (d->head_dim == 128) {
            if (!a.causal) hipLaunchKernelGGL((attn_fwd8_k<128, false, 1>), g8, dim3(512), 0, st, a);
            else if (hpb == 4 && g_attn_opt[2]) hipLaunchKernelGGL((attn_fwd8_k<128, true, 4, 2, true>), g8, dim3(512), 0, st, a);
            else if (hpb == 4) hipLaunchKernelGGL((attn_fwd8_k<128, true, 4>), g8, dim3(512), 0, st, a);
            else if (hpb == 2) hipLaunchKernelGGL((attn_fwd8_k<128, true, 2>), g8, dim3(512), 0, st, a);
            else hipLaunchKernelGGL((attn_fwd8_k<128, true, 1>), g8, dim3(512), 0, st, a);
        } else {
            if (!a.causal && g_attn_opt[1]) hipLaunchKernelGGL((attn_fwd8_k<64, false, 1, 4, false>), g8, dim3(512), 0, st, a);
            else if (!a.causal && g_attn_opt[2]) hipLaunchKernelGGL((attn_fwd8_k<64, false, 1, 2, true>), g8, dim3(512), 0, st, a);
            else if (!a.causal) hipLaunchKernelGGL((attn_fwd8_k<64, false, 1>), g8, dim3(512), 0, st, a);
            else if (hpb == 2) hipLaunchKernelGGL((attn_fwd8_k<64, true, 2>), g8, dim3(512), 0, st, a);
            else hipLaunchKernelGGL((attn_fwd8_k<64, true, 1>), g8, dim3(512), 0, st, a);
        }
        DESTA_CHECK_LAUNCH("attention_fwd");
        return DESTA_OK;
    }
    const bool two = d->head_dim == 64 && a.Sq <= 64;
    dim3 grid((unsigned)((a.Sq + (two ? 63 : 127)) / (two ? 64 : 128)) * a.Hq * a.B);
    if (d->head_dim == 128) hipLaunchKernelGGL((attn_fwd_k<128, false>), grid, dim3(256), 0, (hipStream_t)stream, a);
    else if (two && a.drop_thresh) hipLaunchKernelGGL((attn_fwd_k<64, true, 2>), grid, dim3(128), 0, (hipStream_t)stream, a);
    else if (two) hipLaunchKernelGGL((attn_fwd_k<64, false, 2>), grid, dim3(128), 0, (hipStream_t)stream, a);
    else if (a.drop_thresh) hipLaunchKernelGGL((attn_fwd_k<64, true>), grid, dim3(256), 0, (hipStream_t)stream, a);
    else hipLaunchKernelGGL((attn_fwd_k<64, false>), grid, dim3(256), 0, (hipStream_t)stream, a);
    DESTA_CHECK_LAUNCH("attention_fwd");
    return DESTA_OK;
}

static_assert(DESTA_ATTN_DECODE_CHUNK % 64 == 0 && DESTA_ATTN_DECODE_CHUNK >= 64, "the decode chunk is a multiple of 64 keys");
namespace {
inline size_t decode_ml_floats(size_t items) { return (2 * items + 3) / 4 * 4; }
}
extern "C" int desta_attention_decode_chunk(void) { return DESTA_ATTN_DECODE_CHUNK; }
extern "C" size_t desta_attention_decode_workspace_bytes(int batch, int n_q_heads, int seq_k, int head_dim) {
    if (batch <= 0 || n_q_heads <= 0 || seq_k <= DESTA_ATTN_DECODE_CHUNK || head_dim <= 0) return 0;
    const size_t nch = ((size_t)seq_k + DESTA_ATTN_DECODE_CHUNK - 1) / DESTA_ATTN_DECODE_CHUNK;
    const size_t items = (size_t)batch * n_q_heads * nch;
    return (decode_ml_floats(items) + items * (size_t)head_dim) * sizeof(float);
}

extern "C" int desta_attention_decode(const desta_attn_desc* d, void* workspace, size_t workspace_bytes, void* stream) {
    DESTA_CHECK_ARG(d, "attention_decode: null descriptor");
    DESTA_CHECK_ARG(d->seq_q == 1, "attention_decode: seq_q %d unsupported (one query row per sequence)", d->seq_q);
    DESTA_CHECK_ARG(d->head_dim == 128, "attention_decode: head_dim %d unsupported (128)", d->head_dim);
    DESTA_CHECK_ARG(!d->causal, "attention_decode: causal must be 0 (the one query row sees every key of [kv_start, seq_k))");
    DESTA_CHECK_ARG(d->dropout_p == 0.f, "attention_decode: dropout_p must be 0");
    DESTA_CHECK_ARG(!d->rope_cos_sin, "attention_decode: rope_cos_sin must be NULL");
    DESTA_CHECK_ARG(!d->O_f32, "attention_decode: O_f32 must be NULL");
    DESTA_CHECK_ARG(!d->dO && !d->dQ, "attention_decode: dO and dQ must be NULL (forward only)");
    AttnArgs a;
    if (int rc = fill_args(d, a)) return rc;
    const int G = a.Hq / a.Hkv;
    DESTA_CHECK_ARG(G <= 8, "attention_decode: group of %d query heads per kv head unsupported (at most 8)", G);
    DESTA_CHECK_ARG(d->O && ((size_t)d->O & 15) == 0 && d->o_batch_stride % 8 == 0,
                    "attention_decode: O must be 16-byte aligned with a batch stride that is a multiple of 8 elements");
    DESTA_CHECK_ARG((((size_t)d->Q | (size_t)d->K | (size_t)d->V) & 15) == 0 && d->q_batch_stride % 8 == 0 &&
                    d->k_batch_stride % 8 == 0 && d->v_batch_stride % 8 == 0,
                    "attention_decode: Q, K, V must be 16-byte aligned with batch strides that are multiples of 8 elements");
    const int nch = (a.Sk + DESTA_ATTN_DECODE_CHUNK - 1) / DESTA_ATTN_DECODE_CHUNK;
    const size_t need = desta_attention_decode_workspace_bytes(a.B, a.Hq, a.Sk, 128);
    DESTA_CHECK_ARG(need == 0 || (workspace && workspace_bytes >= need && ((size_t)workspace & 15) == 0),
                    "attention_decode: workspace of %zu bytes is too small or misaligned (%zu needed, 16-byte aligned)", workspace_bytes, need);
    DESTA_CHECK_ARG((long)a.B * a.Hkv * nch <= 0x7fffffffL, "attention_decode: grid too large");
    float* ws_ml = (float*)workspace;
    float* ws_o = ws_ml ? ws_ml + decode_ml_floats((size_t)a.B * a.Hq * nch) : nullptr;
    const dim3 grid((unsigned)(a.B * a.Hkv * nch));
    hipStream_t st = (hipStream_t)stream;
    if (G == 1) hipLaunchKernelGGL((attn_decode_k<1>), grid, dim3(256), 0, st, a, ws_ml, ws_o, nch);
    else if (G == 2) hipLaunchKernelGGL((attn_decode_k<2>), grid, dim3(256), 0, st, a, ws_ml, ws_o, nch);
    else if (G <= 4) hipLaunchKernelGGL((attn_decode_k<4>), grid, dim3(256), 0, st, a, ws_ml, ws_o, nch);
    else hipLaunchKernelGGL((attn_decode_k<8>), grid, dim3(256), 0, st, a, ws_ml, ws_o, nch);
    DESTA_CHECK_LAUNCH("attention_decode");
    if (nch > 1) {
        hipLaunchKernelGGL(attn_decode_combine_k, dim3((unsigned)((a.B * a.Hq + 7) / 8)), dim3(256), 0, st, a, ws_ml, ws_o, nch);
        DESTA_CHECK_LAUNCH("attention_decode (combine)");
    }
    return DESTA_OK;
}

extern "C" int desta_attention_decode_kv8(const desta_attn_desc* d, const float* k_scale, const float* v_scale, int64_t scale_batch_stride,
                                          int64_t scale_row_stride, void* workspace, size_t workspace_bytes, void* stream) {
    DESTA_CHECK_ARG(d, "attention_decode_kv8: null descriptor");
    DESTA_CHECK_ARG(k_scale && v_scale && scale_batch_stride >= 0 && scale_row_stride > 0, "attention_decode_kv8: null scale or bad scale stride");
    DESTA_CHECK_ARG(d->seq_q == 1, "attention_decode_kv8: seq_q %d unsupported (one query row per sequence)", d->seq_q);
    DESTA_CHECK_ARG(d->head_dim == 128, "attention_decode_kv8: head_dim %d unsupported (128)", d->head_dim);
    DESTA_CHECK_ARG(!d->causal, "attention_decode_kv8: causal must be 0 (the one query row sees every key of [kv_start, seq_k))");
    DESTA_CHECK_ARG(d->dropout_p == 0.f, "attention_decode_kv8: dropout_p must be 0");
    DESTA_CHECK_ARG(!d->rope_cos_sin, "attention_decode_kv8: rope_cos_sin must be NULL");
    DESTA_CHECK_ARG(!d->O_f32, "attention_decode_kv8: O_f32 must be NULL");
    DESTA_CHECK_ARG(!d->dO && !d->dQ, "attention_decode_kv8: dO and dQ must be NULL (forward only)");
    AttnArgs a;
    if (int rc = fill_args(d, a)) return rc;
    const int G = a.Hq / a.Hkv;
    DESTA_CHECK_ARG(G <= 8, "attention_decode_kv8: group of %d query heads per kv head unsupported (at most 8)", G);
    DESTA_CHECK_ARG(d->O && ((size_t)d->O & 15) == 0 && d->o_batch_stride % 8 == 0,
                    "attention_decode_kv8: O must be 16-byte aligned with a batch stride that is a multiple of 8 elements");
    DESTA_CHECK_ARG((((size_t)d->Q | (size_t)d->K | (size_t)d->V) & 15) == 0 && d->q_batch_stride % 8 == 0 &&
                    d->k_batch_stride % 8 == 0 && d->v_batch_stride % 8 == 0,
                    "attention_decode_kv8: Q, K, V must be 16-byte aligned with batch strides that are multiples of 8 elements");
    const int nch = (a.Sk + DESTA_ATTN_DECODE_CHUNK - 1) / DESTA_ATTN_DECODE_CHUNK;
    const size_t need = desta_attention_decode_workspace_bytes(a.B, a.Hq, a.Sk, 128);
    DESTA_CHECK_ARG(need == 0 || (workspace && workspace_bytes >= need && ((size_t)workspace & 15) == 0),
                    "attention_decode_kv8: workspace of %zu bytes is too small or misaligned (%zu needed, 16-byte aligned)", workspace_bytes, need);
    DESTA_CHECK_ARG((long)a.B * a.Hkv * nch <= 0x7fffffffL, "attention_decode_kv8: grid too large");
    float* ws_ml = (float*)workspace;
    float* ws_o = ws_ml ? ws_ml + decode_ml_floats((size_t)a.B * a.Hq * nch) : nullptr;
    const dim3 grid((unsigned)(a.B * a.Hkv * nch));
    hipStream_t st = (hipStream_t)stream;
    const long sbs = (long)scale_batch_stride, srs = (long)scale_row_stride;
    if (G == 1) hipLaunchKernelGGL((attn_kv8_k<1>), grid, dim3(256), 0, st, a, k_scale, v_scale, sbs, srs, ws_ml, ws_o, nch);
    else if (G == 2) hipLaunchKernelGGL((attn_kv8_k<2>), grid, dim3(256), 0, st, a, k_scale, v_scale, sbs, srs, ws_ml, ws_o, nch);
    else if (G <= 4) hipLaunchKernelGGL((attn_kv8_k<4>), grid, dim3(256), 0, st, a, k_scale, v_scale, sbs, srs, ws_ml, ws_o, nch);
    else hipLaunchKernelGGL((attn_kv8_k<8>), grid, dim3(256), 0, st, a, k_scale, v_scale, sbs, srs, ws_ml, ws_o, nch);
    DESTA_CHECK_LAUNCH("attention_decode_kv8");
    if (nch > 1) {
        hipLaunchKernelGGL(attn_decode_combine_k, dim3((unsigned)((a.B * a.Hq + 7) / 8)), dim3(256), 0, st, a, ws_ml, ws_o, nch);
        DESTA_CHECK_LAUNCH("attention_decode_kv8 (combine)");
    }
    return DESTA_OK;
}

namespace {
constexpr int KV8_DQ_SLOTS = 16;
__global__ __launch_bounds__(256) void kv8_dequant_k(const uint8_t* __restrict__ cache, long c_bs, long c_rs, const float* __restrict__ scale,
                                                     long s_bs, long s_rs, const int* __restrict__ kv_start, int n_heads, int slot1,
                                                     bf16_t* __restrict__ out, long o_bs, long o_rs) {
    const int b = blockIdx.y;
    const int kv_lo = kv_start ? max(0, min(kv_start[b], slot1)) : 0;
    const int first = max((int)blockIdx.x * KV8_DQ_SLOTS, kv_lo), last = min((int)blockIdx.x * KV8_DQ_SLOTS + KV8_DQ_SLOTS, slot1);
    if (first >= last) return;
    const int per = n_heads * 8;
    const int items = (last - first) * per;
    cache += (long)b * c_bs;
    scale += (long)b * s_bs;
    out += (long)b * o_bs;
    for (int i = threadIdx.x; i < items; i += 256) {
        const int s = first + i / per, r = i % per;
        const uint4 q = *(const uint4*)(cache + (long)s * c_rs + 16 * r);
        const float sc = scale[(long)s * s_rs + (r >> 3)];
        union { bf16x8 v; u16x8 u; } lo, hi;
        lo.v = e4m3x8_to_bf16(make_uint2(q.x, q.y));
        hi.v = e4m3x8_to_bf16(make_uint2(q.z, q.w));
#pragma unroll
        for (int e = 0; e < 8; ++e) {
            lo.u[e] = f2bf(bf2f(lo.u[e]) * sc);
            hi.u[e] = f2bf(bf2f(hi.u[e]) * sc);
        }
        bf16_t* o = out + (long)s * o_rs + 16 * r;
        *(u16x8*)o = lo.u;
        *(u16x8*)(o + 8) = hi.u;
    }
}
}

extern "C" int desta_kv8_dequant(const uint8_t* kv_cache, int64_t kv_batch_stride, int64_t kv_row_stride, const float* kv_scale,
                                 int64_t scale_batch_stride, int64_t scale_row_stride, const int32_t* kv_start, int batch, int n_heads,
                                 int head_dim, int slot1, void* out_bf16, int64_t out_batch_stride, int64_t out_row_stride, void* stream) {
    DESTA_CHECK_ARG(kv_cache && kv_scale && out_bf16, "kv8_dequant: null cache, scale or output");
    DESTA_CHECK_ARG(head_dim == 128, "kv8_dequant: head_dim %d unsupported (128)", head_dim);
    DESTA_CHECK_ARG(batch > 0 && batch <= 65535 && n_heads > 0 && n_heads <= 4096, "kv8_dequant: bad batch %d or n_heads %d", batch, n_heads);
    DESTA_CHECK_ARG(slot1 > 0, "kv8_dequant: slot1 %d must be positive", slot1);
    const long w = (long)n_heads * 128;
    DESTA_CHECK_ARG(((size_t)kv_cache & 15) == 0 && kv_row_stride >= w && kv_row_stride % 16 == 0 && kv_batch_stride >= 0 && kv_batch_stride % 16 == 0,
                    "kv8_dequant: cache must be 16-byte aligned with row / batch strides that are multiples of 16 bytes, rows of at least %ld", w);
    DESTA_CHECK_ARG(scale_row_stride >= n_heads && scale_batch_stride >= 0, "kv8_dequant: bad scale stride");
    DESTA_CHECK_ARG(((size_t)out_bf16 & 15) == 0 && out_row_stride >= w && out_row_stride % 8 == 0 && out_batch_stride >= 0 && out_batch_stride % 8 == 0,
                    "kv8_dequant: output must be 16-byte aligned with row / batch strides that are multiples of 8 elements, rows of at least %ld", w);
    const dim3 grid((unsigned)((slot1 + KV8_DQ_SLOTS - 1) / KV8_DQ_SLOTS), (unsigned)batch);
    hipLaunchKernelGGL(kv8_dequant_k, grid, dim3(256), 0, (hipStream_t)stream, kv_cache, (long)kv_batch_stride, (long)kv_row_stride, kv_scale,
                       (long)scale_batch_stride, (long)scale_row_stride, (const int*)kv_start, n_heads, slot1, (bf16_t*)out_bf16,
                       (long)out_batch_stride, (long)out_row_stride);
    DESTA_CHECK_LAUNCH("kv8_dequant");
    return DESTA_OK;
}

#define ATTN_Q64_MAX_CHUNKS 4
extern "C" size_t desta_attention_bwd_workspace_floats(int batch, int n_q_heads, int seq_q) {
    const size_t delta = ((size_t)batch * n_q_heads * seq_q + 3) / 4 * 4;
    return delta + (seq_q <= 64 ? (size_t)ATTN_Q64_MAX_CHUNKS * batch * n_q_heads * (4096 + 128) : 0);
}

namespace {
struct BwdFork { hipStream_t side = nullptr; hipEvent_t fork = nullptr, join = nullptr; int handles = 0; };
BwdFork g_bwd_fork[16];
std::mutex g_bwd_fork_mu;
int g_bwd_concurrent = 1;
BwdFork* bwd_fork_locked(int dev) {
    BwdFork& f = g_bwd_fork[dev];
    if (!f.side) {
        hipStream_t s = nullptr; hipEvent_t e0 = nullptr, e1 = nullptr;
        if (hipStreamCreateWithFlags(&s, hipStreamNonBlocking) != hipSuccess) return nullptr;
        if (hipEventCreateWithFlags(&e0, hipEventDisableTiming) != hipSuccess ||
            hipEventCreateWithFlags(&e1, hipEventDisableTiming) != hipSuccess) {
            if (e0) (void)hipEventDestroy(e0);
            (void)hipStreamDestroy(s);
            return nullptr;
        }
        f.fork = e0; f.join = e1; f.side = s;
    }
    return &f;
}
BwdFork* bwd_fork() {
    int dev = 0;
    if (hipGetDevice(&dev) != hipSuccess || dev < 0 || dev >= 16) return nullptr;
    if (g_bwd_fork[dev].side) return &g_bwd_fork[dev];
    std::lock_guard<std::mutex> lk(g_bwd_fork_mu);
    return bwd_fork_locked(dev);
}
}
extern "C" int desta_attention_set_concurrent_bwd(int on) { g_bwd_concurrent = on; return DESTA_OK; }
int desta_internal_reserve(void) {
    int dev = 0;
    if (hipGetDevice(&dev) != hipSuccess || dev < 0 || dev >= 16) return DESTA_EINVAL;
    std::lock_guard<std::mutex> lk(g_bwd_fork_mu);
    BwdFork* f = bwd_fork_locked(dev);
    if (!f) return DESTA_ELAUNCH;
    ++f->handles;
    return DESTA_OK;
}
int desta_internal_release(void) {
    int dev = 0;
    if (hipGetDevice(&dev) != hipSuccess || dev < 0 || dev >= 16) return DESTA_EINVAL;
    std::lock_guard<std::mutex> lk(g_bwd_fork_mu);
    BwdFork& f = g_bwd_fork[dev];
    if (f.handles > 0 && --f.handles > 0) return DESTA_OK;
    if (f.side) { (void)hipStreamSynchronize(f.side); (void)hipStreamDestroy(f.side); }
    if (f.fork) (void)hipEventDestroy(f.fork);
    if (f.join) (void)hipEventDestroy(f.join);
    f = BwdFork();
    return DESTA_OK;
}

extern "C" int desta_attention_bwd(const desta_attn_desc* d, float* workspace, void* stream) {
    AttnArgs a;
    if (int rc = fill_args(d, a)) return rc;
    DESTA_CHECK_ARG(d->O && d->dO && d->lse && workspace && d->dQ, "attention_bwd: null argument");
    DESTA_CHECK_ARG((d->dK == nullptr) == (d->dV == nullptr), "attention_bwd: dK and dV go together");
    DESTA_CHECK_ARG(d->dq_row_stride % 4 == 0 && d->do_row_stride % 8 == 0 && d->o_row_stride % 8 == 0,
                    "attention_bwd: bad strides");
    a.delta = workspace;
    hipStream_t st = (hipStream_t)stream;
    const long rows = (long)a.B * a.Hq * a.Sq;
    const int G = d->head_dim / 8;
    dim3 gd((unsigned)((rows * G + 255) / 256));
    dim3 gk_((unsigned)((a.Sk + 127) / 128) * a.Hkv * a.B);
    if (a.rope_cs)
        DESTA_CHECK_ARG(g_attn_opt[0] && !g_attn_opt[3] && !a.drop_thresh && !a.O32 && a.Sq >= 128 && a.Sq == a.Sk && d->dq_row_stride % 8 == 0 &&
                        d->dq_batch_stride % 8 == 0 && ((size_t)d->dQ & 15) == 0 &&
                        (!d->dK || ((((d->dk_row_stride | d->dv_row_stride | d->dk_batch_stride | d->dv_batch_stride) & 7) == 0) &&
                                    (((size_t)d->dK | (size_t)d->dV) & 15) == 0)),
                        "attention_bwd: rope_cos_sin needs seq_q == seq_k >= 128, no dropout and 16-byte aligned dQ / dK / dV");
    if (g_attn_opt[0] && !g_attn_opt[3] && !a.drop_thresh && !a.O32 && a.Sq >= 128 && d->dq_row_stride % 8 == 0 && d->dq_batch_stride % 8 == 0 &&
        ((size_t)d->dQ & 15) == 0) {
        const int G = a.Hq / a.Hkv;
        const int hpb = !a.causal ? 1 : (d->head_dim == 128 ? (G % 4 == 0 ? 4 : (G % 2 == 0 ? 2 : 1)) : (G % 2 == 0 ? 2 : 1));
        const int rb = 256 / hpb;
        dim3 g8((unsigned)((a.Sq + rb - 1) / rb) * (unsigned)(G / hpb) * (unsigned)(a.B * a.Hkv));
        if (d->head_dim == 128) {
            if (!a.causal) hipLaunchKernelGGL((attn_bwd_dq8_k<128, false, 1>), g8, dim3(512), 0, st, a, workspace);
            else if (hpb == 4) hipLaunchKernelGGL((attn_bwd_dq8_k<128, true, 4>), g8, dim3(512), 0, st, a, workspace);
            else if (hpb == 2) hipLaunchKernelGGL((attn_bwd_dq8_k<128, true, 2>), g8, dim3(512), 0, st, a, workspace);
            else hipLaunchKernelGGL((attn_bwd_dq8_k<128, true, 1>), g8, dim3(512), 0, st, a, workspace);
            if (d->dK) {
                if (g_attn_opt[5] && a.causal) {
                    dim3 gk2((unsigned)((a.Sk + 63) / 64) * a.Hkv * a.B);
                    hipLaunchKernelGGL((attn_bwd_dkdv_k<128, false, 2>), gk2, dim3(128), 0, st, a);
                } else hipLaunchKernelGGL((attn_bwd_dkdv_k<128, false>), gk_, dim3(256), 0, st, a);
            }
        } else {
            if (!a.causal) hipLaunchKernelGGL((attn_bwd_dq8_k<64, false, 1>), g8, dim3(512), 0, st, a, workspace);
            else if (hpb == 2) hipLaunchKernelGGL((attn_bwd_dq8_k<64, true, 2>), g8, dim3(512), 0, st, a, workspace);
            else hipLaunchKernelGGL((attn_bwd_dq8_k<64, true, 1>), g8, dim3(512), 0, st, a, workspace);
            if (d->dK) hipLaunchKernelGGL((attn_bwd_dkdv_k<64, false>), gk_, dim3(256), 0, st, a);
        }
        DESTA_CHECK_LAUNCH("attention_bwd");
        return DESTA_OK;
    }
    const bool q64 = d->head_dim == 64 && a.Sq <= 64 && a.Sk >= 256 && !a.causal && a.Hq == a.Hkv && d->dK && !a.rope_cs &&
                     ((d->q_batch_stride | d->k_batch_stride | d->v_batch_stride | d->do_batch_stride) & 7) == 0 && ((size_t)d->dO & 15) == 0 &&
                     (d->dq_batch_stride & 3) == 0 && ((size_t)d->dQ & 7) == 0;
    if (d->dkv_transposed)
        DESTA_CHECK_ARG(q64 && a.Sk % 4 == 0 && d->dkv_t_ld % 4 == 0 && d->dkv_t_ld >= (int64_t)a.B * a.Sk && (((size_t)d->dK | (size_t)d->dV) & 7) == 0,
                        "attention_bwd: dkv_transposed needs the one-query-tile path (head_dim 64, seq_q <= 64, seq_k >= 256 and a multiple of 4, no GQA) and 8-byte aligned dK / dV");
    if ((g_attn_opt[4] || d->dkv_transposed) && q64 &&
        (d->dkv_transposed || (((d->dk_row_stride | d->dv_row_stride | d->dk_batch_stride | d->dv_batch_stride) & 7) == 0 && (((size_t)d->dK | (size_t)d->dV) & 15) == 0))) {
        hipLaunchKernelGGL(attn_delta_k<64>, gd, dim3(256), 0, st, a, workspace);
        const int nkb = (a.Sk + 127) / 128;
        const int nch = nkb >= 8 ? ATTN_Q64_MAX_CHUNKS : (nkb >= 4 ? 2 : 1), bpc = (nkb + nch - 1) / nch;
        float* part = workspace + (rows + 3) / 4 * 4;
        float* bpart = d->dkv_bias_grad ? part + (size_t)ATTN_Q64_MAX_CHUNKS * a.B * a.Hq * 4096 : nullptr;
        dim3 gf((unsigned)(nch * a.B * a.Hq));
        if (d->dkv_transposed) {
            if (a.drop_thresh) hipLaunchKernelGGL((attn_bwd_q64_k<true, true>), gf, dim3(256), 0, st, a, part, bpart, bpc);
            else hipLaunchKernelGGL((attn_bwd_q64_k<false, true>), gf, dim3(256), 0, st, a, part, bpart, bpc);
            if (bpart) hipLaunchKernelGGL(attn_bias_sum_k, dim3((unsigned)(2 * a.Hq)), dim3(256), 0, st, (const float*)bpart,
                                          nch * a.B, 2 * a.Hq * 64, d->dkv_bias_grad);
        } else if (a.drop_thresh) hipLaunchKernelGGL((attn_bwd_q64_k<true, false>), gf, dim3(256), 0, st, a, part, bpart, bpc);
        else hipLaunchKernelGGL((attn_bwd_q64_k<false, false>), gf, dim3(256), 0, st, a, part, bpart, bpc);
        hipLaunchKernelGGL(attn_dq_sum_k, dim3((unsigned)(a.B * a.Hq)), dim3(256), 0, st, a, (const float*)part, nch);
        DESTA_CHECK_LAUNCH("attention_bwd");
        return DESTA_OK;
    }
    const bool two_q = d->head_dim == 64 && a.Sq <= 64;
    dim3 gq((unsigned)((a.Sq + (two_q ? 63 : 127)) / (two_q ? 64 : 128)) * a.Hq * a.B);
    dim3 gk((unsigned)((a.Sk + 127) / 128) * a.Hkv * a.B);
    if (d->head_dim == 128) {
        hipLaunchKernelGGL(attn_delta_k<128>, gd, dim3(256), 0, st, a, workspace);
        BwdFork* f = (g_bwd_concurrent && d->dK) ? bwd_fork() : nullptr;
        if (f && hipEventRecord(f->fork, st) == hipSuccess && hipStreamWaitEvent(f->side, f->fork, 0) == hipSuccess) {
            hipLaunchKernelGGL((attn_bwd_dkdv_k<128, false>), gk, dim3(256), 0, st, a);
            hipLaunchKernelGGL((attn_bwd_dq_k<128, false>), gq, dim3(256), 0, f->side, a);
            DESTA_CHECK_ARG(hipEventRecord(f->join, f->side) == hipSuccess && hipStreamWaitEvent(st, f->join, 0) == hipSuccess,
                            "attention_bwd: could not join the side stream");
        } else {
            hipLaunchKernelGGL((attn_bwd_dq_k<128, false>), gq, dim3(256), 0, st, a);
            if (d->dK) hipLaunchKernelGGL((attn_bwd_dkdv_k<128, false>), gk, dim3(256), 0, st, a);
        }
    } else {
        hipLaunchKernelGGL(attn_delta_k<64>, gd, dim3(256), 0, st, a, workspace);
        const bool two = two_q;
        if (a.drop_thresh) {
            if (two) hipLaunchKernelGGL((attn_bwd_dq_k<64, true, 2>), gq, dim3(128), 0, st, a);
            else hipLaunchKernelGGL((attn_bwd_dq_k<64, true>), gq, dim3(256), 0, st, a);
            if (d->dK) hipLaunchKernelGGL((attn_bwd_dkdv_k<64, true>), gk, dim3(256), 0, st, a);
        } else {
            if (two) hipLaunchKernelGGL((attn_bwd_dq_k<64, false, 2>), gq, dim3(128), 0, st, a);
            else hipLaunchKernelGGL((attn_bwd_dq_k<64, false>), gq, dim3(256), 0, st, a);
            if (d->dK) hipLaunchKernelGGL((attn_bwd_dkdv_k<64, false>), gk, dim3(256), 0, st, a);
        }
    }
    DESTA_CHECK_LAUNCH("attention_bwd");
    return DESTA_OK;
}
```

### desta2.5-audio_amd/desta/_hip.py

```python
from __future__ import annotations

import ctypes as C
import os

import torch

_HERE = os.path.dirname(os.path.abspath(__file__))
LIB_PATH = os.environ.get("DESTA_HIP_LIB") or os.path.join(_HERE, "lib", "libdesta_hip.so")

if not os.path.exists(LIB_PATH):
    raise ImportError(
        f"{LIB_PATH} is missing: build it with `python desta2.5-audio_amd/build.py` "
        "(hipcc --offload-arch=gfx950). There is no CPU/eager fallback for the DeSTA2.5 hot path.")

lib = C.CDLL(LIB_PATH, mode=C.RTLD_GLOBAL)

vp, i32, i64, f32 = C.c_void_p, C.c_int, C.c_int64, C.c_float


class GemmDesc(C.Structure):
    _fields_ = [("A", vp), ("B", vp), ("C", vp),
                ("M", i32), ("N", i32), ("K", i32), ("batch", i32),
                ("lda", i64), ("ldb", i64), ("ldc", i64),
                ("stride_a", i64), ("stride_b", i64), ("stride_c", i64),
# ... 419 lines not shown


def tap_mix_bwd(x, lw, dout, taps, batch, prompt, d, dx, dlw):
    check(_mix_bwd(p(x), p(lw), p(dout), taps, batch, prompt, d, p(dx), p(dlw), stream()), "desta_tap_mix_bwd")


class AttnDesc(C.Structure):
    _fields_ = [("Q", vp), ("K", vp), ("V", vp), ("O", vp), ("dO", vp), ("dQ", vp), ("dK", vp), ("dV", vp),
                ("lse", vp),
                ("q_batch_stride", i64), ("q_row_stride", i64), ("k_batch_stride", i64), ("k_row_stride", i64),
                ("v_batch_stride", i64), ("v_row_stride", i64), ("o_batch_stride", i64), ("o_row_stride", i64),
                ("do_batch_stride", i64), ("do_row_stride", i64), ("dq_batch_stride", i64), ("dq_row_stride", i64),
                ("dk_batch_stride", i64), ("dk_row_stride", i64), ("dv_batch_stride", i64), ("dv_row_stride", i64),
                ("batch", i32), ("n_q_heads", i32), ("n_kv_heads", i32), ("seq_q", i32), ("seq_k", i32),
                ("head_dim", i32), ("causal", i32), ("kv_start", vp), ("scale", f32),
                ("dropout_p", f32), ("dropout_seed", C.c_uint64), ("rope_cos_sin", vp), ("O_f32", vp),
                ("dkv_transposed", i32), ("dkv_t_ld", i64), ("dkv_bias_grad", vp)]


_attn_fwd = _sig("desta_attention_fwd", C.POINTER(AttnDesc), vp)
lib.desta_attention_bwd_workspace_floats.restype = c_size_t
lib.desta_attention_bwd_workspace_floats.argtypes = [i32, i32, i32]
_attn_bwd = _sig("desta_attention_bwd", C.POINTER(AttnDesc), vp, vp)


def _elem_ptr(t, offset_elems):
    return t.data_ptr() + offset_elems * t.element_size()


def attn_desc(q, k, v, o, lse, *, batch, hq, hkv, sq, sk, hd, scale, causal=False, kv_start=None,
              q_off=0, k_off=0, v_off=0, q_rs=None, k_rs=None, v_rs=None, o_rs=None, dropout_p=0.0, dropout_seed=0,
              q_bs=None, k_bs=None, v_bs=None, o_bs=None, o_f32=None):
    d = AttnDesc()
    q_rs = q.shape[-1] if q_rs is None else q_rs
    k_rs = k.shape[-1] if k_rs is None else k_rs
    v_rs = v.shape[-1] if v_rs is None else v_rs
    o_rs = o.shape[-1] if o_rs is None else o_rs
    d.Q, d.K, d.V, d.O = _elem_ptr(q, q_off), _elem_ptr(k, k_off), _elem_ptr(v, v_off), p(o)
    d.lse = p(lse)
    d.q_row_stride, d.q_batch_stride = q_rs, (sq * q_rs if q_bs is None else q_bs)
    d.k_row_stride, d.k_batch_stride = k_rs, (sk * k_rs if k_bs is None else k_bs)
    d.v_row_stride, d.v_batch_stride = v_rs, (sk * v_rs if v_bs is None else v_bs)
    d.o_row_stride, d.o_batch_stride = o_rs, (sq * o_rs if o_bs is None else o_bs)
    d.batch, d.n_q_heads, d.n_kv_heads, d.seq_q, d.seq_k, d.head_dim = batch, hq, hkv, sq, sk, hd
    d.causal = int(causal)
    d.kv_start = p(kv_start)
    d.scale = scale
    d.dropout_p, d.dropout_seed = dropout_p, dropout_seed
    if o_f32 is not None:
        assert o_f32.dtype == torch.float32 and o_f32.shape == o.shape and o_f32.is_contiguous() and o.is_contiguous()
    d.O_f32 = p(o_f32)
    d._keep = (q, k, v, o, lse, kv_start, o_f32)
    return d


def _attn_flops(d, mult):
    f = 4.0 * d.batch * d.n_q_heads * d.seq_q * d.seq_k * d.head_dim
    return mult * (f * 0.5 if d.causal else f)


def _attn_tag(d, *a, **k):
    return f"D{d.head_dim}{'c' if d.causal else ''}_q{d.seq_q}_k{d.seq_k}"


@_profiled(lambda d: "attn_fwd:" + _attn_tag(d), lambda d: _attn_flops(d, 1.0))
def attention_fwd(d: AttnDesc):
    check(_attn_fwd(C.byref(d), stream()), "desta_attention_fwd")


lib.desta_attention_decode_chunk.restype = i32
lib.desta_attention_decode_workspace_bytes.restype = c_size_t
lib.desta_attention_decode_workspace_bytes.argtypes = [i32, i32, i32, i32]
_attn_decode = _sig("desta_attention_decode", C.POINTER(AttnDesc), vp, c_size_t, vp)
DECODE_ATTN_CHUNK = int(lib.desta_attention_decode_chunk())
DECODE_ATTN_MIN_KEYS = 448
ATTN_DECODE_CALLS = 0


def attention_decode_workspace_bytes(batch: int, hq: int, sk: int, hd: int = 128) -> int:
    return int(lib.desta_attention_decode_workspace_bytes(int(batch), int(hq), int(sk), int(hd)))


@_profiled(lambda d, *a, **k: "attn_decode:" + _attn_tag(d), lambda d, *a, **k: _attn_flops(d, 1.0))
def attention_decode(d: AttnDesc, ws=None):
    global ATTN_DECODE_CALLS
    check(_attn_decode(C.byref(d), p(ws), 0 if ws is None else ws.numel() * ws.element_size(), stream()), "desta_attention_decode")
    ATTN_DECODE_CALLS += 1


_attn_kv8 = _sig("desta_attention_decode_kv8", C.POINTER(AttnDesc), vp, vp, i64, i64, vp, c_size_t, vp)
ATTN_KV8_CALLS = 0


@_profiled(lambda d, *a, **k: "attn_kv8:" + _attn_tag(d), lambda d, *a, **k: _attn_flops(d, 1.0))
def attention_decode_kv8(d: AttnDesc, k_scale, v_scale, scale_bs, scale_rs, ws=None):
    global ATTN_KV8_CALLS
    check(_attn_kv8(C.byref(d), p(k_scale), p(v_scale), int(scale_bs), int(scale_rs), p(ws),
                    0 if ws is None else ws.numel() * ws.element_size(), stream()), "desta_attention_decode_kv8")
    ATTN_KV8_CALLS += 1


_kv8_dequant = _sig("desta_kv8_dequant", vp, i64, i64, vp, i64, i64, vp, i32, i32, i32, i32, vp, i64, i64, vp)
KV8_DEQUANT_CALLS = 0


@_profiled("kv8_dequant", lambda *a, **k: 3.0 * a[7] * a[10] * a[8] * a[9])
def kv8_dequant(cache, kv_bs, kv_rs, scale, scale_bs, scale_rs, kv_start, batch, n_heads, hd, slot1, out, out_bs, out_rs):
    global KV8_DEQUANT_CALLS
    check(_kv8_dequant(p(cache), int(kv_bs), int(kv_rs), p(scale), int(scale_bs), int(scale_rs), p(kv_start), int(batch), int(n_heads),
                       int(hd), int(slot1), p(out), int(out_bs), int(out_rs), stream()), "desta_kv8_dequant")
    KV8_DEQUANT_CALLS += 1


@_profiled(lambda d, *a, **k: "attn_bwd:" + _attn_tag(d), lambda d, *a, **k: _attn_flops(d, 2.5))
def attention_bwd(d: AttnDesc, do, dq, dk=None, dv=None, *, do_rs=None, dq_off=0, dk_off=0, dv_off=0, dq_rs=None,
                  dk_rs=None, dv_rs=None, do_bs=None, dq_bs=None, dk_bs=None, dv_bs=None, rope_cos_sin=None, dkv_t=None):
    d.rope_cos_sin = p(rope_cos_sin)
    d._keep_rope = rope_cos_sin
    do_rs = do.shape[-1] if do_rs is None else do_rs
    dq_rs = dq.shape[-1] if dq_rs is None else dq_rs
    d.dO, d.do_row_stride, d.do_batch_stride = p(do), do_rs, (d.seq_q * do_rs if do_bs is None else do_bs)
    d.dQ, d.dq_row_stride, d.dq_batch_stride = _elem_ptr(dq, dq_off), dq_rs, (d.seq_q * dq_rs if dq_bs is None else dq_bs)
    d.dkv_transposed, d.dkv_t_ld, d.dkv_bias_grad = 0, 0, 0
    if dkv_t is not None:
        t, ld, bias = dkv_t
        assert dk is None and dv is None and t.dtype == torch.bfloat16 and (bias is None or bias.dtype == torch.float32)
        d.dK, d.dV = p(t), _elem_ptr(t, d.n_q_heads * d.head_dim * ld)
        d.dkv_transposed, d.dkv_t_ld, d.dkv_bias_grad = 1, ld, p(bias)
        dk = dv = t
    elif dk is not None:
        dk_rs = dk.shape[-1] if dk_rs is None else dk_rs
        dv_rs = dv.shape[-1] if dv_rs is None else dv_rs
        d.dK, d.dk_row_stride, d.dk_batch_stride = _elem_ptr(dk, dk_off), dk_rs, (d.seq_k * dk_rs if dk_bs is None else dk_bs)
        d.dV, d.dv_row_stride, d.dv_batch_stride = _elem_ptr(dv, dv_off), dv_rs, (d.seq_k * dv_rs if dv_bs is None else dv_bs)
    else:
        d.dK = d.dV = 0
    ws = scratch(lib.desta_attention_bwd_workspace_floats(d.batch, d.n_q_heads, d.seq_q), do.device, "attn")
    d._keep_bwd = (do, dq, dk, dv, ws)
    check(_attn_bwd(C.byref(d), p(ws), stream()), "desta_attention_bwd")


_prompt_expand = _sig("desta_prompt_expand", vp, i32, i32, i64, vp, vp, vp)
_prompt_grad = _sig("desta_prompt_grad", vp, i32, i32, i64, vp, vp)


def prompt_expand(prompts, taps, batch, n, x32, x16):
    check(_prompt_expand(p(prompts), taps, batch, n, p(x32), p(x16), stream()), "desta_prompt_expand")


def prompt_grad(dx, taps, batch, n, dprompts):
    check(_prompt_grad(p(dx), taps, batch, n, p(dprompts), stream()), "desta_prompt_grad")


def gemm_force_variant(v: int) -> None:
    lib.desta_gemm_force_variant.argtypes = [i32]
    lib.desta_gemm_force_variant(v)


_dropout = _sig("desta_dropout_bf16", vp, vp, i32, i32, i64, f32, C.c_uint64, vp)
_dropout_mask = _sig("desta_dropout_mask_u8", C.c_uint64, i64, f32, vp, vp)


def dropout_bf16(x, y, rows, cols, ld, p_drop, seed):
    check(_dropout(p(x), p(y), rows, cols, ld, p_drop, seed, stream()), "desta_dropout_bf16")


def dropout_mask(seed, n, p_drop, device="cuda"):
    out = torch.empty(n, dtype=torch.uint8, device=device)
    check(_dropout_mask(seed, n, p_drop, p(out), stream()), "desta_dropout_mask_u8")
    return out


def gemm_set_persistent(on: bool) -> None:
    lib.desta_gemm_set_persistent.argtypes = [i32]
    lib.desta_gemm_set_persistent(int(on))


def gemm_set_option(option: int, value: int) -> None:
    lib.desta_gemm_set_option.argtypes = [i32, i32]
    check(lib.desta_gemm_set_option(option, value), "desta_gemm_set_option")


_argmax = _sig("desta_argmax_bf16", vp, i64, i32, i32, vp, vp, vp)
lib.desta_argmax_workspace_bytes.restype = C.c_size_t
lib.desta_argmax_workspace_bytes.argtypes = [i32]
_argmax_ws = {}


def argmax_bf16(x, ld, rows, cols, out):
    key = (x.device, rows)
    ws = _argmax_ws.get(key)
    if ws is None:
        ws = _argmax_ws[key] = torch.empty(lib.desta_argmax_workspace_bytes(rows), dtype=torch.uint8, device=x.device)
    check(_argmax(p(x), ld, rows, cols, p(out), p(ws), stream()), "desta_argmax_bf16")


_mask_tokens = _sig("desta_mask_tokens_bf16", vp, i64, i32, i32, vp, i32, vp)


def mask_tokens_bf16(logits, ld, rows, cols, ids):
    check(_mask_tokens(p(logits), ld, rows, cols, p(ids), int(ids.numel()), stream()), "desta_mask_tokens_bf16")


_rope_kv = _sig("desta_rope_kv_append", vp, i64, i32, i32, i32, i32, i32, vp, vp, vp, f32, vp, vp, i64, i64, i32, vp)


def rope_kv_append(buf, ld, rows, seq, n_q, n_kv, hd, cos_sin, q_norm_w, k_norm_w, eps, pos_shift, cache, kv_bs, kv_rs, slot0):
    check(_rope_kv(p(buf), ld, rows, seq, n_q, n_kv, hd, p(cos_sin), p(q_norm_w), p(k_norm_w), eps, p(pos_shift), p(cache), kv_bs,
                   kv_rs, slot0, stream()), "desta_rope_kv_append")


_rope_kv8 = _sig("desta_rope_kv_append_e4m3", vp, i64, i32, i32, i32, i32, i32, vp, vp, vp, f32, vp, vp, i64, i64, vp, i64, i64, i32, vp)


def rope_kv_append_e4m3(buf, ld, rows, seq, n_q, n_kv, hd, cos_sin, q_norm_w, k_norm_w, eps, pos_shift, cache, kv_bs, kv_rs,
                        scale, scale_bs, scale_rs, slot0):
    check(_rope_kv8(p(buf), ld, rows, seq, n_q, n_kv, hd, p(cos_sin), p(q_norm_w), p(k_norm_w), eps, p(pos_shift), p(cache), kv_bs,
                    kv_rs, p(scale), scale_bs, scale_rs, slot0, stream()), "desta_rope_kv_append_e4m3")


_sample = _sig("desta_sample_top_p_bf16", vp, i64, i32, i32, f32, f32, C.c_uint64, C.c_uint32, vp, vp, vp)


def sample_top_p(logits, ld, rows, cols, temperature, top_p, seed, step, out, keep_mask=None):
    check(_sample(p(logits), ld, rows, cols, temperature, top_p, seed & 0xFFFFFFFFFFFFFFFF, step & 0xFFFFFFFF, p(out), p(keep_mask),
                  stream()), "desta_sample_top_p_bf16")


_sample_chain = _sig("desta_sample_bf16", vp, i64, i32, i32, vp, i64, i32, f32, i32, f32, i32, f32, f32, C.c_uint64, C.c_uint32,
                     vp, vp, vp)


def sample(logits, ld, rows, cols, out, *, do_sample=True, temperature=1.0, top_k=0, top_p=1.0, min_p=0.0, repetition_penalty=1.0,
           hist=None, hist_len=0, seed=0, step=0, keep_mask=None):
    hist_ld = 0 if hist is None else hist.stride(0)
    check(_sample_chain(p(logits), ld, rows, cols, p(hist), hist_ld, hist_len, repetition_penalty, int(bool(do_sample)), temperature,
                        top_k, top_p, min_p, seed & 0xFFFFFFFFFFFFFFFF, step & 0xFFFFFFFF, p(out), p(keep_mask), stream()),
          "desta_sample_bf16")


class CommUniqueId(C.Structure):
    _fields_ = [("internal", C.c_char * 128)]


def comm_get_unique_id() -> bytes:
    lib.desta_comm_get_unique_id.argtypes = [C.POINTER(CommUniqueId)]
    uid = CommUniqueId()
    check(lib.desta_comm_get_unique_id(C.byref(uid)), "desta_comm_get_unique_id")
    return bytes(C.string_at(C.addressof(uid), 128))


def comm_create(world_size: int, rank: int, unique_id: bytes) -> int:
    lib.desta_comm_create.argtypes = [C.POINTER(vp), i32, i32, C.POINTER(CommUniqueId)]
    uid = CommUniqueId()
    C.memmove(C.addressof(uid), unique_id, 128)
    comm = vp()
    check(lib.desta_comm_create(C.byref(comm), world_size, rank, C.byref(uid)), "desta_comm_create")
    return comm.value


def allreduce_grads(comm: int, grads: torch.Tensor) -> None:
    assert grads.dtype == torch.float32 and grads.is_contiguous()
    lib.desta_allreduce_grads.argtypes = [vp, vp, i64, vp]
    check(lib.desta_allreduce_grads(comm, p(grads), grads.numel(), stream()), "desta_allreduce_grads")


def comm_destroy(comm: int) -> None:
    lib.desta_comm_destroy.argtypes = [vp]
    check(lib.desta_comm_destroy(comm), "desta_comm_destroy")


class Context:

    def __init__(self, device: int = 0):
        lib.desta_create.argtypes = [i32, C.POINTER(vp)]
        h = vp()
        check(lib.desta_create(int(device), C.byref(h)), "desta_create")
        self.handle = h.value

    def info(self) -> dict:
        lib.desta_handle_info.argtypes = [vp, C.POINTER(i32), C.POINTER(i32), C.c_char_p, C.c_size_t]
        dev, cus, arch = i32(), i32(), C.create_string_buffer(64)
        check(lib.desta_handle_info(self.handle, C.byref(dev), C.byref(cus), arch, 64), "desta_handle_info")
        return {"device": dev.value, "compute_units": cus.value, "arch": arch.value.decode()}

    def last_error(self) -> str:
        lib.desta_handle_last_error.argtypes = [vp]
        lib.desta_handle_last_error.restype = C.c_char_p
        return lib.desta_handle_last_error(self.handle).decode()

    def close(self) -> None:
        if self.handle:
            lib.desta_destroy.argtypes = [vp]
            check(lib.desta_destroy(self.handle), "desta_destroy")
            self.handle = None

    def __enter__(self):
        return self

    def __exit__(self, *exc):
        self.close()


def attention_set_option(which: int, value: int) -> None:
    lib.desta_attention_set_option.argtypes = [i32, i32]
    check(lib.desta_attention_set_option(int(which), int(value)), "desta_attention_set_option")


def attention_set_concurrent_bwd(on: bool) -> None:
    lib.desta_attention_set_concurrent_bwd.argtypes = [i32]
    check(lib.desta_attention_set_concurrent_bwd(int(on)), "desta_attention_set_concurrent_bwd")


def _check_struct_layouts() -> None:
    lib.desta_sizeof_desc.restype = C.c_size_t
    lib.desta_sizeof_desc.argtypes = [i32]
    for which, cls in ((0, GemmDesc), (1, AttnDesc), (2, OptPlan), (3, AdamWPlan)):
        if lib.desta_sizeof_desc(which) != C.sizeof(cls):
            raise ImportError(f"struct layout mismatch for {cls.__name__}: library {lib.desta_sizeof_desc(which)} B, binding {C.sizeof(cls)} B")


_check_struct_layouts()


_scatter = _sig("desta_scatter_rows_bf16", vp, vp, i32, i32, vp, vp)
_target_rows = _sig("desta_target_rows", vp, i32, i32, vp, vp, vp, i32, vp)


def scatter_rows(src, idx, rows, hidden, out):
    check(_scatter(p(src), p(idx), rows, hidden, p(out), stream()), "desta_scatter_rows_bf16")


def target_rows(labels, batch, seq, idx, compact_labels, count, s_major=False):
    check(_target_rows(p(labels), batch, seq, p(idx), p(compact_labels), p(count), int(s_major), stream()), "desta_target_rows")


_orca_local_mix = _sig("desta_orca_local_mix", vp, vp, i32, i64, i32, vp, vp)
_orca_rope = _sig("desta_orca_rope", vp, vp, i32, i32, i32, C.c_float, C.c_float, i32, vp)
_orca_gate_residual = _sig("desta_orca_gate_residual", vp, i64, vp, vp, vp, vp, i64, i32, i32, vp, vp)
_orca_sim_loss = _sig("desta_orca_sim_loss", vp, vp, vp, i32, i32, i32, i64, i32, i32, vp, vp)
_orca_align = _sig("desta_orca_align", vp, i32, vp, i64, i64, i32, vp, i32, vp, vp)


def orca_local_mix(x, layer_weights, taps, rows, d, out):
    check(_orca_local_mix(p(x), p(layer_weights), taps, rows, d, p(out), stream()), "desta_orca_local_mix")


def orca_rope(x, y, batch, tokens, hidden, theta, position_scale, round_cos_sin=True):
    check(_orca_rope(p(x), p(y), batch, tokens, hidden, float(theta), float(position_scale), int(round_cos_sin), stream()), "desta_orca_rope")


def orca_gate_residual(hidden, ld_hidden, cross, gate_hidden, gate_w2, gate_b2, rows, hidden_size, gate_width, gate_out=None):
    check(_orca_gate_residual(p(hidden), ld_hidden, p(cross), p(gate_hidden), p(gate_w2), p(gate_b2), rows, hidden_size, gate_width,
                              p(gate_out), stream()), "desta_orca_gate_residual")


def orca_sim_loss(x, y, y_index, batch, nx, ny, y_rows, hidden, subtract_identity, partials):
    check(_orca_sim_loss(p(x), p(y), p(y_index), batch, nx, ny, y_rows, hidden, int(subtract_identity), p(partials), stream()), "desta_orca_sim_loss")


def orca_align(audio, tokens, hidden, row_stride, batch_stride, hidden_size, spans, n_spans, out):
    check(_orca_align(p(audio), tokens, p(hidden), row_stride, batch_stride, hidden_size, p(spans), n_spans, p(out), stream()), "desta_orca_align")


_orca_gate_residual_bwd = _sig("desta_orca_gate_residual_bwd", vp, i64, vp, vp, i64, i32, vp, vp, vp)
_orca_gate_mlp_bwd = _sig("desta_orca_gate_mlp_bwd", vp, vp, vp, vp, i64, i32, vp, vp, vp, vp, vp)
_orca_align_bwd = _sig("desta_orca_align_bwd", vp, i32, vp, i64, i64, i32, vp, i32, C.c_float, vp, i64, i64, vp)
_orca_rope_bwd = _sig("desta_orca_rope_bwd", vp, i32, i32, i32, C.c_float, C.c_float, i32, i32, vp, vp, vp)
_orca_col2im_add = _sig("desta_orca_col2im_add", vp, i32, i32, i32, i32, i32, i32, vp, vp)
_orca_local_mix_bwd = _sig("desta_orca_local_mix_bwd", vp, vp, vp, i32, i64, i32, vp, vp, vp)
_orca_sim_loss_bwd = _sig("desta_orca_sim_loss_bwd", vp, vp, i64, vp, vp, i64, i32, i32, i32, i32, i32, C.c_float, vp, vp)


def orca_gate_residual_bwd(d_out, ld, cross, gate, rows, hidden_size, d_cross, d_gate_pre):
    check(_orca_gate_residual_bwd(p(d_out), ld, p(cross), p(gate), rows, hidden_size, p(d_cross), p(d_gate_pre), stream()), "desta_orca_gate_residual_bwd")


_gate_ws: dict = {}


def orca_gate_mlp_bwd(d_gate_pre, gate_preact, gate_hidden, gate_w2, rows, gate_width, d_preact, d_w2, d_b2):
    key = (d_gate_pre.device, gate_width)
    if key not in _gate_ws:
        _gate_ws[key] = torch.empty(64 * (gate_width + 1), dtype=torch.float32, device=d_gate_pre.device)
    check(_orca_gate_mlp_bwd(p(d_gate_pre), p(gate_preact), p(gate_hidden), p(gate_w2), rows, gate_width, p(d_preact), p(d_w2), p(d_b2), p(_gate_ws[key]),
                             stream()), "desta_orca_gate_mlp_bwd")


def orca_align_bwd(audio, tokens, hidden, row_stride, batch_stride, hidden_size, spans, n_spans, coef, d_hidden, d_row_stride, d_batch_stride):
    check(_orca_align_bwd(p(audio), tokens, p(hidden), row_stride, batch_stride, hidden_size, p(spans), n_spans, float(coef), p(d_hidden), d_row_stride,
                          d_batch_stride, stream()), "desta_orca_align_bwd")


def orca_rope_bwd(d_rotated, batch, tokens, hidden, theta, position_scale, round_cos_sin, n_first, d_first, d_rest):
    check(_orca_rope_bwd(p(d_rotated), batch, tokens, hidden, float(theta), float(position_scale), int(round_cos_sin), n_first, p(d_first), p(d_rest), stream()),
          "desta_orca_rope_bwd")


def orca_col2im_add(d_col, batch, tokens_out, tokens_padded, hidden, kernel, stride, d_padded):
    check(_orca_col2im_add(p(d_col), batch, tokens_out, tokens_padded, hidden, kernel, stride, p(d_padded), stream()), "desta_orca_col2im_add")


def orca_local_mix_bwd(d_out, x, layer_weights, taps, rows, d, d_layer_weights):
    ws = scratch(256 * 32, d_out.device, tag="orca_mix")
    check(_orca_local_mix_bwd(p(d_out), p(x), p(layer_weights), taps, rows, d, p(d_layer_weights), p(ws), stream()), "desta_orca_local_mix_bwd")


def orca_sim_loss_bwd(x, x_index, x_rows, y, y_index, y_rows, batch, nx, ny, hidden, subtract_identity, coef, d_x):
    check(_orca_sim_loss_bwd(p(x), p(x_index), x_rows, p(y), p(y_index), y_rows, batch, nx, ny, hidden, int(subtract_identity), float(coef), p(d_x), stream()),
          "desta_orca_sim_loss_bwd")
```

Before: 6.485.

## Add persistent work-queue scheduling to causal head-dim-128 attention forward kernel

Adds a persistent variant of the causal head-dim-128 forward attention kernel. It launches CUs times occupancy blocks, and each block pulls further (batch, head-group, q-block) items from per-XCD atomic counters, prefetching the next item's first K/V tile and Q while it finishes the current one. The aim is to cut tail imbalance and block launch/ramp-up cost for causal attention, where item costs vary widely. In exchange it adds atomics, a device-global queue table keyed by stream, and a depart counter that resets the queue. It is enabled by default (option 6 = 1) only when there are more items than the persistent grid. The dq backward kernel gets the same plumbing, but its launches still pass a null queue.

```diff
diff --git a/desta2.5-audio_amd/csrc/attention.hip b/desta2.5-audio_amd/csrc/attention.hip
--- a/desta2.5-audio_amd/csrc/attention.hip
+++ b/desta2.5-audio_amd/csrc/attention.hip
@@ -334,51 +334,96 @@
     return __builtin_shufflevector(a, c, 0, 1, 2, 3, 4, 5, 6, 7);
 }
 
-template <int D, bool CAUSAL, int HPB, int MINW = 2, bool STAGGER = false>
-__global__ __launch_bounds__(512, MINW) void attn_fwd8_k(AttnArgs p) {
+struct AttnItem {
+    int b, h, q0, qcol, kv_lo, t_lo, t_hi, q_abs, wave_kmax;
+    bool wave_on;
+    const char *kbase, *vbase;
+};
+template <int D, bool CAUSAL, int HPB>
+__device__ __forceinline__ AttnItem attn_item(const AttnArgs& p, const int id, const int wave, const int lane) {
+    constexpr int RB = 256 / HPB, WPH = RB / 32;
+    const int G = p.Hq / p.Hkv, nq = (p.Sq + RB - 1) / RB, hgroups = G / HPB, ngrp = p.B * p.Hkv, coff = p.Sk - p.Sq;
+    AttnItem it;
+    int g, qblk, hg;
+    const int per = nq * hgroups;
+    if ((ngrp & 7) == 0) {
+        const int xcd = id & 7, slot = id >> 3, gpx = ngrp >> 3;
+        if (CAUSAL) {
+            const int r = slot % (hgroups * gpx);
+            qblk = nq - 1 - slot / (hgroups * gpx); hg = r / gpx; g = (r % gpx) * 8 + xcd;
+        } else {
+            const int r = slot % per;
+            g = (slot / per) * 8 + xcd; hg = r / nq; qblk = r % nq;
+        }
+    } else if (CAUSAL) {
+        const int r = id % (hgroups * ngrp);
+        qblk = nq - 1 - id / (hgroups * ngrp); hg = r / ngrp; g = r % ngrp;
+    } else {
+        const int r = id % per;
+        g = id / per; hg = r / nq; qblk = r % nq;
+    }
+    const int hk = g % p.Hkv, qb0 = qblk * RB;
+    it.b = g / p.Hkv;
+    it.h = hk * G + hg * HPB + wave / WPH;
+    it.q0 = qb0 + (wave % WPH) * 32;
+    it.qcol = it.q0 + (lane & 31);
+    it.wave_on = it.q0 < p.Sq;
+    it.kv_lo = p.kv_start ? max(0, min(p.kv_start[it.b], p.Sk)) : 0;
+    int kv_hi = p.Sk;
+    if (CAUSAL) kv_hi = min(p.Sk, min(qb0 + RB - 1, p.Sq - 1) + coff + 1);
+    it.t_lo = it.kv_lo / 64; it.t_hi = (kv_hi + 63) / 64;
+    it.q_abs = it.qcol + coff;
+    it.wave_kmax = CAUSAL ? min(it.q0 + 31, p.Sq - 1) + coff : p.Sk - 1;
+    it.kbase = (const char*)(p.K + (long)it.b * p.k_bs + (long)hk * D);
+    it.vbase = (const char*)(p.V + (long)it.b * p.v_bs + (long)hk * D);
+    return it;
+}
+__device__ __forceinline__ int attn_draw_ahead(int* counter, int wave) {
+    const unsigned lane_mask = __builtin_amdgcn_readfirstlane(wave == 0 ? 1u : 0u);
+    unsigned long saved;
+    int nxt;
+    asm volatile("s_mov_b64 %1, exec\n\t"
+                 "s_mov_b32 exec_lo, %3\n\t"
+                 "s_mov_b32 exec_hi, 0\n\t"
+                 "global_atomic_add %0, %2, %4, off sc0\n\t"
+                 "s_mov_b64 exec, %1"
+                 : "=&v"(nxt), "=&s"(saved) : "v"(counter), "s"(lane_mask), "v"(1) : "memory");
+    return nxt;
+}
+__device__ __forceinline__ void attn_depart(int* queue) {
+    asm volatile("s_waitcnt vmcnt(0)" ::: "memory");
+    __syncthreads();
+    if (threadIdx.x == 0) {
+        const int dpt = __hip_atomic_fetch_add(queue + 8, 1, __ATOMIC_RELAXED, __HIP_MEMORY_SCOPE_AGENT);
+        if (dpt == (int)gridDim.x - 1) {
+#pragma unroll
+            for (int k = 0; k < 9; ++k) __hip_atomic_store(queue + k, 0, __ATOMIC_RELAXED, __HIP_MEMORY_SCOPE_AGENT);
+        }
+    }
+}
+
+template <int D, bool CAUSAL, int HPB, int MINW = 2, bool STAGGER = false, bool PERSIST = false>
+__global__ __launch_bounds__(512, MINW) void attn_fwd8_k(AttnArgs p, int* __restrict__ queue) {
+    static_assert(!(PERSIST && STAGGER), "the persistent form is built for the lockstep schedule");
     constexpr int NT = 512, RB = 256 / HPB, WPH = RB / 32;
     constexpr int TILE = 64 * D * 2;
     constexpr int SLOT = 2 * TILE, NSLOT = STAGGER ? 3 : 2;
     constexpr int NCH = 64 * (D / 8) / NT;
-    __shared__ __attribute__((aligned(16))) char lds[NSLOT * SLOT];
+    __shared__ __attribute__((aligned(16))) char lds[NSLOT * SLOT + (PERSIST ? 16 : 0)];
     const int lane = threadIdx.x & 63, wave = __builtin_amdgcn_readfirstlane(threadIdx.x >> 6), h2 = lane >> 5;
     const int G = p.Hq / p.Hkv, nq = (p.Sq + RB - 1) / RB, hgroups = G / HPB, ngrp = p.B * p.Hkv;
-    int g, qblk, hg;
-    {
-        const int id = blockIdx.x, per = nq * hgroups;
-        if ((ngrp & 7) == 0) {
-            const int xcd = id & 7, slot = id >> 3, gpx = ngrp >> 3;
-            if (CAUSAL) {
-                const int r = slot % (hgroups * gpx);
-                qblk = nq - 1 - slot / (hgroups * gpx); hg = r / gpx; g = (r % gpx) * 8 + xcd;
-            } else {
-                const int r = slot % per;
-                g = (slot / per) * 8 + xcd; hg = r / nq; qblk = r % nq;
-            }
-        } else if (CAUSAL) {
-            const int r = id % (hgroups * ngrp);
-            qblk = nq - 1 - id / (hgroups * ngrp); hg = r / ngrp; g = r % ngrp;
-        } else {
-            const int r = id % per;
-            g = id / per; hg = r / nq; qblk = r % nq;
-        }
-    }
-    const int b = g / p.Hkv, hk = g % p.Hkv;
-    const int h = hk * G + hg * HPB + wave / WPH;
-    const int qb0 = qblk * RB, q0 = qb0 + (wave % WPH) * 32;
-    const int qcol = q0 + (lane & 31);
-    const bool wave_on = q0 < p.Sq;
-
     const int coff = p.Sk - p.Sq;
-    const int kv_lo = p.kv_start ? max(0, min(p.kv_start[b], p.Sk)) : 0;
-    int kv_hi = p.Sk;
-    if (CAUSAL) kv_hi = min(p.Sk, min(qb0 + RB - 1, p.Sq - 1) + coff + 1);
-    const int t_lo = kv_lo / 64, t_hi = (kv_hi + 63) / 64;
-    const int q_abs = qcol + coff;
-    const int wave_kmax = CAUSAL ? min(q0 + 31, p.Sq - 1) + coff : p.Sk - 1;
-
-    const char* kbase = (const char*)(p.K + (long)b * p.k_bs + (long)hk * D);
-    const char* vbase = (const char*)(p.V + (long)b * p.v_bs + (long)hk * D);
+    auto geometry = [&](const int id) __attribute__((always_inline)) { return attn_item<D, CAUSAL, HPB>(p, id, wave, lane); };
+    int* const s_ticket = (int*)(lds + NSLOT * SLOT);
+    const int nitems = nq * hgroups * ngrp;
+    const int nqueue = min(8, (int)gridDim.x), xq = (int)blockIdx.x % nqueue;
+    const int qblocks = ((int)gridDim.x - xq + nqueue - 1) / nqueue;
+    int* const counter = queue + xq;
+    auto ticket_item = [&]() { return (qblocks + __builtin_amdgcn_readfirstlane(*s_ticket)) * nqueue + xq; };
+    bool have = !PERSIST || (int)blockIdx.x < nitems;
+    AttnItem cur = {}, nx = {};
+    if (have) cur = geometry(blockIdx.x);
+
     int srow[NCH], sdst[NCH];
     unsigned ksrc[NCH], vsrc[NCH];
 #pragma unroll
@@ -391,9 +436,9 @@
     }
     typedef typename stage_vec<NCH>::type stage8_t;
     stage8_t kr = {}, vr = {};
-    auto load_tile = [&](const int kt) __attribute__((always_inline)) {
-        const char* kb_ = kbase + (long)kt * 64 * p.k_rs * 2;
-        const char* vb_ = vbase + (long)kt * 64 * p.v_rs * 2;
+    auto load_tile = [&](const AttnItem& it, const int kt) __attribute__((always_inline)) {
+        const char* kb_ = it.kbase + (long)kt * 64 * p.k_rs * 2;
+        const char* vb_ = it.vbase + (long)kt * 64 * p.v_rs * 2;
         const bool ragged = kt * 64 + 64 > p.Sk;
 #pragma unroll
         for (int i = 0; i < NCH; ++i) {
@@ -416,15 +461,16 @@
         }
     };
 
-    load_tile(t_lo);
-    const bf16_t* qptr = p.Q + (long)b * p.q_bs + (long)min(qcol, p.Sq - 1) * p.q_rs + (long)h * D;
     bf16x8 qf[D / 16];
-#pragma unroll
-    for (int ds = 0; ds < D / 16; ++ds) qf[ds] = *(const bf16x8*)(qptr + 16 * ds + 8 * h2);
-#pragma unroll
-    for (int ds = 0; ds < D / 16; ++ds) asm volatile("" :: "v"(qf[ds]));
-    store_tile(lds);
-    load_tile(t_lo + 1);
+    auto load_q = [&](const AttnItem& it) __attribute__((always_inline)) {
+        const bf16_t* qptr = p.Q + (long)it.b * p.q_bs + (long)min(it.qcol, p.Sq - 1) * p.q_rs + (long)it.h * D;
+#pragma unroll
+        for (int ds = 0; ds < D / 16; ++ds) qf[ds] = *(const bf16x8*)(qptr + 16 * ds + 8 * h2);
+    };
+    if (have) {
+        load_tile(cur, cur.t_lo);
+        load_q(cur);
+    }
 
     int kofs[D / 16], vofs[D / 32][2];
 #pragma unroll
@@ -444,17 +490,17 @@
     }
 
     f32x16 oacc[D / 32];
-#pragma unroll
-    for (int i = 0; i < D / 32; ++i)
-#pragma unroll
-        for (int r = 0; r < 16; ++r) oacc[i][r] = 0.f;
-    float m = -INFINITY, l = 0.f;
+    float m, l;
     f32x16 st[2];
+    int nxt = 0;
 #define ATTN_BARRIER() asm volatile("s_waitcnt lgkmcnt(0)\n\ts_barrier" ::: "memory")
-    ATTN_BARRIER();
+    auto hand_off = [&]() __attribute__((always_inline)) {
+        asm volatile("s_waitcnt vmcnt(0)" ::: "memory");
+        if (threadIdx.x == 0) *s_ticket = nxt;
+    };
 
     auto scores = [&](const int kt, const int sb) __attribute__((always_inline)) {
-        if (!(wave_on && kt * 64 <= wave_kmax)) return;
+        if (!(cur.wave_on && kt * 64 <= cur.wave_kmax)) return;
 #pragma unroll
         for (int kb = 0; kb < 2; ++kb)
 #pragma unroll
@@ -474,7 +520,7 @@
         __builtin_amdgcn_sched_barrier(0);
 #pragma unroll
         for (int ds = 0; ds < D / 16; ++ds) st[1] = __builtin_amdgcn_mfma_f32_32x32x16_bf16(kbf[ds], qf[ds], st[1], 0, 0, 0);
-        const bool need_mask = (kt * 64 + 63 >= p.Sk) || (kt * 64 < kv_lo) || (CAUSAL && kt * 64 + 63 > q0 + coff);
+        const bool need_mask = (kt * 64 + 63 >= p.Sk) || (kt * 64 < cur.kv_lo) || (CAUSAL && kt * 64 + 63 > cur.q0 + coff);
         if (need_mask) {
             asm volatile("; boundary tile" ::: "memory");
 #pragma unroll
@@ -482,7 +528,7 @@
 #pragma unroll
                 for (int r = 0; r < 16; ++r) {
                     const int key = kt * 64 + kb * 32 + acc_row(r, lane);
-                    const bool ok = key < p.Sk && key >= kv_lo && (!CAUSAL || key <= q_abs);
+                    const bool ok = key < p.Sk && key >= cur.kv_lo && (!CAUSAL || key <= cur.q_abs);
                     st[kb][r] = ok ? st[kb][r] : -INFINITY;
                 }
         }
@@ -512,7 +558,7 @@
             }
     };
     auto pv = [&](const int kt, const int sb) __attribute__((always_inline)) {
-        if (!(wave_on && kt * 64 <= wave_kmax)) return;
+        if (!(cur.wave_on && kt * 64 <= cur.wave_kmax)) return;
         int vad[D / 32][2];
 #pragma unroll
         for (int i = 0; i < D / 32; ++i)
@@ -530,14 +576,60 @@
             }
     };
     auto stage = [&](const int kt, const int sb_next) __attribute__((always_inline)) {
-        if (kt + 1 < t_hi) {
+        if (kt + 1 < cur.t_hi) {
             store_tile(lds + sb_next);
-            if (kt + 2 < t_hi) load_tile(kt + 2);
+            if (kt + 2 < cur.t_hi) load_tile(cur, kt + 2);
         }
     };
     auto next_slot = [](int sb) { return sb == (NSLOT - 1) * SLOT ? 0 : sb + SLOT; };
+    bool have_nx = false;
+    auto take_ticket = [&]() __attribute__((always_inline)) {
+        const int id = ticket_item();
+        have_nx = id < nitems;
+        if (have_nx) {
+            nx = geometry(id);
+            load_tile(nx, nx.t_lo);
+        }
+    };
+    while (have) {
+    const int t_lo = cur.t_lo, t_hi = cur.t_hi;
+#pragma unroll
+    for (int ds = 0; ds < D / 16; ++ds) asm volatile("" :: "v"(qf[ds]));
+    store_tile(lds);
+    load_tile(cur, t_lo + 1);
+#pragma unroll
+    for (int i = 0; i < D / 32; ++i)
+#pragma unroll
+        for (int r = 0; r < 16; ++r) oacc[i][r] = 0.f;
+    m = -INFINITY; l = 0.f;
+    ATTN_BARRIER();
+
     int sb = 0;
-    if (!STAGGER || wave < 4) {
+    if (PERSIST) {
+        for (int kt = t_lo; kt + 1 < t_hi; ++kt) {
+            const int sn = next_slot(sb);
+            if (kt + 2 == t_hi) nxt = attn_draw_ahead(counter, wave);
+            scores(kt, sb);
+            stage(kt, sn);
+            pv(kt, sb);
+            if (kt + 2 == t_hi) hand_off();
+            ATTN_BARRIER();
+            sb = sn;
+        }
+        const bool early = t_hi - t_lo >= 2;
+        if (early) take_ticket();
+        else if (threadIdx.x == 0) *s_ticket = __hip_atomic_fetch_add(counter, 1, __ATOMIC_RELAXED, __HIP_MEMORY_SCOPE_AGENT);
+        if (t_lo < t_hi) {
+            scores(t_hi - 1, sb);
+            if (early && have_nx) load_q(nx);
+            pv(t_hi - 1, sb);
+        }
+        ATTN_BARRIER();
+        if (!early) {
+            take_ticket();
+            if (have_nx) load_q(nx);
+        }
+    } else if (!STAGGER || wave < 4) {
         for (int kt = t_lo; kt < t_hi; ++kt) {
             const int sn = next_slot(sb);
             scores(kt, sb);
@@ -560,12 +652,11 @@
         }
         pv(t_hi - 1, sb);
     }
-#undef ATTN_BARRIER
-
-    if (wave_on && qcol < p.Sq) {
+
+    if (cur.wave_on && cur.qcol < p.Sq) {
         const float lt = swap_halves_sum(l);
         const float inv = lt > 0.f ? 1.0f / lt : 0.f;
-        bf16_t* optr = p.O + (long)b * p.o_bs + (long)qcol * p.o_rs + (long)h * D;
+        bf16_t* optr = p.O + (long)cur.b * p.o_bs + (long)cur.qcol * p.o_rs + (long)cur.h * D;
 #pragma unroll
         for (int i = 0; i < D / 32; ++i)
 #pragma unroll
@@ -581,15 +672,21 @@
                 *(uint4*)(optr + i * 32 + 16 * j + 8 * h2) = make_uint4(r0[0], r1[0], r0[1], r1[1]);
             }
         if (p.O32) {
-            float* o32 = p.O32 + (long)b * p.o_bs + (long)qcol * p.o_rs + (long)h * D;
+            float* o32 = p.O32 + (long)cur.b * p.o_bs + (long)cur.qcol * p.o_rs + (long)cur.h * D;
 #pragma unroll
             for (int i = 0; i < D / 32; ++i)
 #pragma unroll
                 for (int rq = 0; rq < 4; ++rq)
                     *(f32x4*)(o32 + i * 32 + 8 * rq + 4 * h2) = f32x4{oacc[i][4 * rq] * inv, oacc[i][4 * rq + 1] * inv, oacc[i][4 * rq + 2] * inv, oacc[i][4 * rq + 3] * inv};
         }
-        if (p.lse && h2 == 0) p.lse[((long)b * p.Hq + h) * p.Sq + qcol] = lt > 0.f ? m + log2f(lt) : INFINITY;
-    }
+        if (p.lse && h2 == 0) p.lse[((long)cur.b * p.Hq + cur.h) * p.Sq + cur.qcol] = lt > 0.f ? m + log2f(lt) : INFINITY;
+    }
+    if (!PERSIST) break;
+    cur = nx;
+    have = have_nx;
+    }
+#undef ATTN_BARRIER
+    if (PERSIST) attn_depart(queue);
 }
 
 template <int D>
@@ -764,50 +861,26 @@
     }
 }
 
-template <int D, bool CAUSAL, int HPB>
-__global__ __launch_bounds__(512, 2) void attn_bwd_dq8_k(AttnArgs p, float* __restrict__ delta_out) {
+template <int D, bool CAUSAL, int HPB, bool PERSIST = false>
+__global__ __launch_bounds__(512, 2) void attn_bwd_dq8_k(AttnArgs p, float* __restrict__ delta_out, int* __restrict__ queue) {
     constexpr int NT = 512, RB = 256 / HPB, WPH = RB / 32;
     constexpr int TILE = 64 * D * 2, SLOT = 2 * TILE;
     constexpr int NCH = 64 * (D / 8) / NT;
-    __shared__ __attribute__((aligned(16))) char lds[2 * SLOT];
+    __shared__ __attribute__((aligned(16))) char lds[2 * SLOT + (PERSIST ? 16 : 0)];
     const int lane = threadIdx.x & 63, wave = __builtin_amdgcn_readfirstlane(threadIdx.x >> 6), h2 = lane >> 5;
     const int G = p.Hq / p.Hkv, nq = (p.Sq + RB - 1) / RB, hgroups = G / HPB, ngrp = p.B * p.Hkv;
-    int g, qblk, hg;
-    {
-        const int id = blockIdx.x, per = nq * hgroups;
-        if ((ngrp & 7) == 0) {
-            const int xcd = id & 7, slot = id >> 3, gpx = ngrp >> 3;
-            if (CAUSAL) {
-                const int r = slot % (hgroups * gpx);
-                qblk = nq - 1 - slot / (hgroups * gpx); hg = r / gpx; g = (r % gpx) * 8 + xcd;
-            } else {
-                const int r = slot % per;
-                g = (slot / per) * 8 + xcd; hg = r / nq; qblk = r % nq;
-            }
-        } else if (CAUSAL) {
-            const int r = id % (hgroups * ngrp);
-            qblk = nq - 1 - id / (hgroups * ngrp); hg = r / ngrp; g = r % ngrp;
-        } else {
-            const int r = id % per;
-            g = id / per; hg = r / nq; qblk = r % nq;
-        }
-    }
-    const int b = g / p.Hkv, hk = g % p.Hkv;
-    const int h = hk * G + hg * HPB + wave / WPH;
-    const int qb0 = qblk * RB, q0 = qb0 + (wave % WPH) * 32;
-    const int qcol = q0 + (lane & 31), qc = min(qcol, p.Sq - 1);
-    const bool wave_on = q0 < p.Sq;
-
     const int coff = p.Sk - p.Sq;
-    const int kv_lo = p.kv_start ? max(0, min(p.kv_start[b], p.Sk)) : 0;
-    int kv_hi = p.Sk;
-    if (CAUSAL) kv_hi = min(p.Sk, min(qb0 + RB - 1, p.Sq - 1) + coff + 1);
-    const int t_lo = kv_lo / 64, t_hi = (kv_hi + 63) / 64;
-    const int q_abs = qcol + coff;
-    const int wave_kmax = CAUSAL ? min(q0 + 31, p.Sq - 1) + coff : p.Sk - 1;
-
-    const char* kbase = (const char*)(p.K + (long)b * p.k_bs + (long)hk * D);
-    const char* vbase = (const char*)(p.V + (long)b * p.v_bs + (long)hk * D);
+    auto geometry = [&](const int id) __attribute__((always_inline)) { return attn_item<D, CAUSAL, HPB>(p, id, wave, lane); };
+    int* const s_ticket = (int*)(lds + 2 * SLOT);
+    const int nitems = nq * hgroups * ngrp;
+    const int nqueue = min(8, (int)gridDim.x), xq = (int)blockIdx.x % nqueue;
+    const int qblocks = ((int)gridDim.x - xq + nqueue - 1) / nqueue;
+    int* const counter = queue + xq;
+    auto ticket_item = [&]() { return (qblocks + __builtin_amdgcn_readfirstlane(*s_ticket)) * nqueue + xq; };
+    bool have = !PERSIST || (int)blockIdx.x < nitems;
+    AttnItem cur = {}, nx = {};
+    if (have) cur = geometry(blockIdx.x);
+
     int srow[NCH], sdst[NCH];
     unsigned ksrc[NCH], vsrc[NCH];
 #pragma unroll
@@ -820,9 +893,9 @@
     }
     typedef typename stage_vec<NCH>::type stage8_t;
     stage8_t kr = {}, vr = {};
-    auto load_tile = [&](const int kt) __attribute__((always_inline)) {
-        const char* kb_ = kbase + (long)kt * 64 * p.k_rs * 2;
-        const char* vb_ = vbase + (long)kt * 64 * p.v_rs * 2;
+    auto load_tile = [&](const AttnItem& it, const int kt) __attribute__((always_inline)) {
+        const char* kb_ = it.kbase + (long)kt * 64 * p.k_rs * 2;
+        const char* vb_ = it.vbase + (long)kt * 64 * p.v_rs * 2;
         const bool ragged = kt * 64 + 64 > p.Sk;
 #pragma unroll
         for (int i = 0; i < NCH; ++i) {
@@ -845,29 +918,41 @@
         }
     };
 
-    load_tile(t_lo);
-    const bf16_t* qptr = p.Q + (long)b * p.q_bs + (long)qc * p.q_rs + (long)h * D;
-    const bf16_t* gptr = p.dO + (long)b * p.do_bs + (long)qc * p.do_rs + (long)h * D;
-    const bf16_t* optr = p.O + (long)b * p.o_bs + (long)qc * p.o_rs + (long)h * D;
-    bf16x8 qf[D / 16], gf[D / 16];
-    float dl = 0.f;
-#pragma unroll
-    for (int ds = 0; ds < D / 16; ++ds) {
-        qf[ds] = *(const bf16x8*)(qptr + 16 * ds + 8 * h2);
-        gf[ds] = *(const bf16x8*)(gptr + 16 * ds + 8 * h2);
-        const bf16x8 of = *(const bf16x8*)(optr + 16 * ds + 8 * h2);
-#pragma unroll
-        for (int j = 0; j < 8; ++j) dl += (float)of[j] * (float)gf[ds][j];
-    }
-    const long stat = ((long)b * p.Hq + h) * p.Sq + qc;
-    const float nlse = -p.lse[stat];
-    const float dlt = swap_halves_sum(dl);
-    if (wave_on && qcol < p.Sq && h2 == 0) delta_out[stat] = dlt;
-#pragma unroll
-    for (int ds = 0; ds < D / 16; ++ds) asm volatile("" :: "v"(qf[ds]), "v"(gf[ds]));
-    asm volatile("" :: "v"(nlse));
-    store_tile(lds);
-    load_tile(t_lo + 1);
+    bf16x8 qf[D / 16], gf[D / 16], of[D / 16];
+    float nlse;
+    long stat;
+    auto load_rows = [&](const AttnItem& it, const bool q_lse, const bool do_o) __attribute__((always_inline)) {
+        const int qc = min(it.qcol, p.Sq - 1);
+        const bf16_t* qptr = p.Q + (long)it.b * p.q_bs + (long)qc * p.q_rs + (long)it.h * D;
+        const bf16_t* gptr = p.dO + (long)it.b * p.do_bs + (long)qc * p.do_rs + (long)it.h * D;
+        const bf16_t* optr = p.O + (long)it.b * p.o_bs + (long)qc * p.o_rs + (long)it.h * D;
+#pragma unroll
+        for (int ds = 0; ds < D / 16; ++ds) {
+            if (q_lse) qf[ds] = *(const bf16x8*)(qptr + 16 * ds + 8 * h2);
+            if (do_o) {
+                gf[ds] = *(const bf16x8*)(gptr + 16 * ds + 8 * h2);
+                of[ds] = *(const bf16x8*)(optr + 16 * ds + 8 * h2);
+            }
+        }
+        if (q_lse) {
+            stat = ((long)it.b * p.Hq + it.h) * p.Sq + qc;
+            nlse = -p.lse[stat];
+        }
+    };
+    float dlt;
+    auto take_delta = [&]() __attribute__((always_inline)) {
+        float dl = 0.f;
+#pragma unroll
+        for (int ds = 0; ds < D / 16; ++ds)
+#pragma unroll
+            for (int j = 0; j < 8; ++j) dl += (float)of[ds][j] * (float)gf[ds][j];
+        dlt = swap_halves_sum(dl);
+        if (cur.wave_on && cur.qcol < p.Sq && h2 == 0) delta_out[stat] = dlt;
+    };
+    if (have) {
+        load_tile(cur, cur.t_lo);
+        load_rows(cur, true, !PERSIST);
+    }
 
     int kofs[D / 16], tofs[D / 32][2];
 #pragma unroll
@@ -886,24 +971,56 @@
         }
     }
     f32x16 dq[D / 32];
+    int nxt = 0;
+#define ATTN_BARRIER() asm volatile("s_waitcnt lgkmcnt(0)\n\ts_barrier" ::: "memory")
+    auto hand_off = [&]() __attribute__((always_inline)) {
+        asm volatile("s_waitcnt vmcnt(0)" ::: "memory");
+        if (threadIdx.x == 0) *s_ticket = nxt;
+    };
+
+    bool have_nx = false;
+    auto take_ticket = [&]() __attribute__((always_inline)) {
+        const int id = ticket_item();
+        have_nx = id < nitems;
+        if (have_nx) {
+            nx = geometry(id);
+            load_tile(nx, nx.t_lo);
+        }
+    };
+    while (have) {
+    const int t_lo = cur.t_lo, t_hi = cur.t_hi;
+    if (PERSIST) {
+        load_rows(cur, false, true);
+#pragma unroll
+        for (int ds = 0; ds < D / 16; ++ds) asm volatile("" :: "v"(qf[ds]));
+    } else {
+        take_delta();
+#pragma unroll
+        for (int ds = 0; ds < D / 16; ++ds) asm volatile("" :: "v"(qf[ds]), "v"(gf[ds]));
+    }
+    asm volatile("" :: "v"(nlse));
+    store_tile(lds);
+    load_tile(cur, t_lo + 1);
+    if (PERSIST) {
+        take_delta();
+#pragma unroll
+        for (int ds = 0; ds < D / 16; ++ds) asm volatile("" :: "v"(gf[ds]));
+    }
 #pragma unroll
     for (int i = 0; i < D / 32; ++i)
 #pragma unroll
         for (int r = 0; r < 16; ++r) dq[i][r] = 0.f;
-#define ATTN_BARRIER() asm volatile("s_waitcnt lgkmcnt(0)\n\ts_barrier" ::: "memory")
     ATTN_BARRIER();
 
-    int sb = 0;
-    for (int kt = t_lo; kt < t_hi; ++kt) {
-        const int sn = SLOT - sb;
-        const bool act = wave_on && kt * 64 <= wave_kmax;
+    auto tile = [&](const int kt, const int sb) __attribute__((always_inline)) {
+        const bool act = cur.wave_on && kt * 64 <= cur.wave_kmax;
         if (act) {
             int kad[D / 16];
 #pragma unroll
             for (int ds = 0; ds < D / 16; ++ds) { kad[ds] = kofs[ds] + sb; asm volatile("" : "+v"(kad[ds])); }
 #pragma unroll
             for (int kb = 0; kb < 2; ++kb) {
-                if (CAUSAL && kt * 64 + kb * 32 > wave_kmax) break;
+                if (CAUSAL && kt * 64 + kb * 32 > cur.wave_kmax) break;
                 f32x16 st, dp;
 #pragma unroll
                 for (int r = 0; r < 16; ++r) { st[r] = 0.f; dp[r] = 0.f; }
@@ -912,14 +1029,14 @@
                     st = __builtin_amdgcn_mfma_f32_32x32x16_bf16(*(const bf16x8*)(lds + kad[ds] + kb * 32 * D * 2), qf[ds], st, 0, 0, 0);
                     dp = __builtin_amdgcn_mfma_f32_32x32x16_bf16(*(const bf16x8*)(lds + kad[ds] + TILE + kb * 32 * D * 2), gf[ds], dp, 0, 0, 0);
                 }
-                const bool need_mask = (kt * 64 + kb * 32 + 31 >= p.Sk) || (kt * 64 + kb * 32 < kv_lo) ||
-                                       (CAUSAL && kt * 64 + kb * 32 + 31 > q0 + coff);
+                const bool need_mask = (kt * 64 + kb * 32 + 31 >= p.Sk) || (kt * 64 + kb * 32 < cur.kv_lo) ||
+                                       (CAUSAL && kt * 64 + kb * 32 + 31 > cur.q0 + coff);
                 if (need_mask) {
                     asm volatile("; boundary tile" ::: "memory");
 #pragma unroll
                     for (int r = 0; r < 16; ++r) {
                         const int key = kt * 64 + kb * 32 + acc_row(r, lane);
-                        const bool ok = key < p.Sk && key >= kv_lo && (!CAUSAL || key <= q_abs);
+                        const bool ok = key < p.Sk && key >= cur.kv_lo && (!CAUSAL || key <= cur.q_abs);
                         st[r] = ok ? st[r] : -INFINITY;
                     }
                 }
@@ -942,19 +1059,45 @@
                 }
             }
         }
+    };
+    auto stage = [&](const int kt, const int sn) __attribute__((always_inline)) {
         if (kt + 1 < t_hi) {
             store_tile(lds + sn);
-            if (kt + 2 < t_hi) load_tile(kt + 2);
-        }
+            if (kt + 2 < t_hi) load_tile(cur, kt + 2);
+        }
+    };
+    int sb = 0;
+    if (PERSIST) {
+        for (int kt = t_lo; kt + 1 < t_hi; ++kt) {
+            const int sn = SLOT - sb;
+            if (kt + 2 == t_hi) nxt = attn_draw_ahead(counter, wave);
+            tile(kt, sb);
+            stage(kt, sn);
+            if (kt + 2 == t_hi) hand_off();
+            ATTN_BARRIER();
+            sb = sn;
+        }
+        const bool early = t_hi - t_lo >= 2;
+        if (early) take_ticket();
+        else if (threadIdx.x == 0) *s_ticket = __hip_atomic_fetch_add(counter, 1, __ATOMIC_RELAXED, __HIP_MEMORY_SCOPE_AGENT);
+        if (t_lo < t_hi) tile(t_hi - 1, sb);
         ATTN_BARRIER();
-        sb = sn;
-    }
-#undef ATTN_BARRIER
-
-    if (wave_on && qcol < p.Sq) {
-        bf16_t* dqp = p.dQ + (long)b * p.dq_bs + (long)qcol * p.dq_rs + (long)h * D;
+        if (!early) take_ticket();
+        if (have_nx) load_rows(nx, true, false);
+    } else {
+        for (int kt = t_lo; kt < t_hi; ++kt) {
+            const int sn = SLOT - sb;
+            tile(kt, sb);
+            stage(kt, sn);
+            ATTN_BARRIER();
+            sb = sn;
+        }
+    }
+
+    if (cur.wave_on && cur.qcol < p.Sq) {
+        bf16_t* dqp = p.dQ + (long)cur.b * p.dq_bs + (long)cur.qcol * p.dq_rs + (long)cur.h * D;
         if (p.rope_cs) {
-            const float* cs = p.rope_cs + (long)qcol * D;
+            const float* cs = p.rope_cs + (long)cur.qcol * D;
 #pragma unroll
             for (int i = 0; i < D / 32; ++i)
 #pragma unroll
@@ -980,6 +1123,12 @@
                 *(uint4*)(dqp + i * 32 + 16 * j + 8 * h2) = make_uint4(r0[0], r1[0], r0[1], r1[1]);
             }
     }
+    if (!PERSIST) break;
+    cur = nx;
+    have = have_nx;
+    }
+#undef ATTN_BARRIER
+    if (PERSIST) attn_depart(queue);
 }
 
 #ifndef ATTN_DKDV_QR
@@ -1892,11 +2041,59 @@
 
 }
 
-namespace { int g_attn_opt[8] = {1, 0, 0, 0, 1, 0, 0, 0}; }
+namespace { int g_attn_opt[8] = {1, 0, 0, 0, 1, 0, 1, 0}; }
 extern "C" int desta_attention_set_option(int which, int value) {
     DESTA_CHECK_ARG(which >= 0 && which < 8, "attention_set_option: unknown option %d", which);
+    DESTA_CHECK_ARG(which != 6 || (value >= 0 && value <= 2), "attention_set_option: option 6 takes 0 (never), 1 (by rule) or 2 (always)");
+    DESTA_CHECK_ARG(which != 7 || value >= 0, "attention_set_option: option 7 takes a block count (0 = no cap)");
     g_attn_opt[which] = value;
     return DESTA_OK;
+}
+
+namespace {
+constexpr int ATTN_QSETS = 64;
+__device__ int g_attn_queues[ATTN_QSETS][16];
+struct AttnQueueTable { int* base = nullptr; int cus = 0; int n = 0; hipStream_t streams[ATTN_QSETS]; };
+AttnQueueTable g_attn_qt[16];
+std::mutex g_attn_qt_mu;
+int* attn_queue_for(hipStream_t st, int& dev, int& cus) {
+    if (hipGetDevice(&dev) != hipSuccess || dev < 0 || dev >= 16) return nullptr;
+    std::lock_guard<std::mutex> lk(g_attn_qt_mu);
+    AttnQueueTable& t = g_attn_qt[dev];
+    if (!t.base) {
+        void* sym = nullptr;
+        int n = 0;
+        if (hipGetSymbolAddress(&sym, HIP_SYMBOL(g_attn_queues)) != hipSuccess || !sym) return nullptr;
+        if (hipDeviceGetAttribute(&n, hipDeviceAttributeMultiprocessorCount, dev) != hipSuccess || n <= 0) return nullptr;
+        t.cus = n; t.base = (int*)sym;
+    }
+    cus = t.cus;
+    for (int i = 0; i < t.n; ++i)
+        if (t.streams[i] == st) return t.base + 16 * i;
+    if (t.n == ATTN_QSETS) return nullptr;
+    t.streams[t.n] = st;
+    return t.base + 16 * t.n++;
+}
+template <auto KERNEL>
+int attn_persistent_grid(int items, hipStream_t st, int*& queue) {
+    static int per_cu[16] = {};
+    queue = nullptr;
+    const int mode = g_attn_opt[6];
+    if (mode == 0) return 0;
+    int dev = 0, cus = 0;
+    int* q = attn_queue_for(st, dev, cus);
+    if (!q) return 0;
+    int bpc = __atomic_load_n(&per_cu[dev], __ATOMIC_RELAXED);
+    if (!bpc) {
+        if (hipOccupancyMaxActiveBlocksPerMultiprocessor(&bpc, KERNEL, 512, 0) != hipSuccess || bpc <= 0) return 0;
+        __atomic_store_n(&per_cu[dev], bpc, __ATOMIC_RELAXED);
+    }
+    int grid = cus * bpc;
+    if (g_attn_opt[7] > 0) grid = min(grid, g_attn_opt[7]);
+    if (mode == 1 && items <= grid) return 0;
+    queue = q;
+    return grid;
+}
 }
 
 extern "C" int desta_attention_fwd(const desta_attn_desc* d, void* stream) {
@@ -1911,18 +2108,28 @@
         const int rb = 256 / hpb;
         dim3 g8((unsigned)((a.Sq + rb - 1) / rb) * (unsigned)(G / hpb) * (unsigned)(a.B * a.Hkv));
         hipStream_t st = (hipStream_t)stream;
+        int* const NOQ = nullptr;
         if (d->head_dim == 128) {
-            if (!a.causal) hipLaunchKernelGGL((attn_fwd8_k<128, false, 1>), g8, dim3(512), 0, st, a);
-            else if (hpb == 4 && g_attn_opt[2]) hipLaunchKernelGGL((attn_fwd8_k<128, true, 4, 2, true>), g8, dim3(512), 0, st, a);
-            else if (hpb == 4) hipLaunchKernelGGL((attn_fwd8_k<128, true, 4>), g8, dim3(512), 0, st, a);
-            else if (hpb == 2) hipLaunchKernelGGL((attn_fwd8_k<128, true, 2>), g8, dim3(512), 0, st, a);
-            else hipLaunchKernelGGL((attn_fwd8_k<128, true, 1>), g8, dim3(512), 0, st, a);
+            if (!a.causal) hipLaunchKernelGGL((attn_fwd8_k<128, false, 1>), g8, dim3(512), 0, st, a, NOQ);
+            else if (hpb == 4 && g_attn_opt[2]) hipLaunchKernelGGL((attn_fwd8_k<128, true, 4, 2, true>), g8, dim3(512), 0, st, a, NOQ);
+            else {
+#define FWD8_LAUNCH(HPB_) do {                                                                                                  \
+                    int* queue = nullptr;                                                                                       \
+                    const int pg = attn_persistent_grid<attn_fwd8_k<128, true, HPB_, 2, false, true>>((int)g8.x, st, queue);    \
+                    if (pg) hipLaunchKernelGGL((attn_fwd8_k<128, true, HPB_, 2, false, true>), dim3(pg), dim3(512), 0, st, a, queue); \
+                    else hipLaunchKernelGGL((attn_fwd8_k<128, true, HPB_>), g8, dim3(512), 0, st, a, NOQ);                      \
+                } while (0)
+                if (hpb == 4) FWD8_LAUNCH(4);
+                else if (hpb == 2) FWD8_LAUNCH(2);
+                else FWD8_LAUNCH(1);
+#undef FWD8_LAUNCH
+            }
         } else {
-            if (!a.causal && g_attn_opt[1]) hipLaunchKernelGGL((attn_fwd8_k<64, false, 1, 4, false>), g8, dim3(512), 0, st, a);
-            else if (!a.causal && g_attn_opt[2]) hipLaunchKernelGGL((attn_fwd8_k<64, false, 1, 2, true>), g8, dim3(512), 0, st, a);
-            else if (!a.causal) hipLaunchKernelGGL((attn_fwd8_k<64, false, 1>), g8, dim3(512), 0, st, a);
-            else if (hpb == 2) hipLaunchKernelGGL((attn_fwd8_k<64, true, 2>), g8, dim3(512), 0, st, a);
-            else hipLaunchKernelGGL((attn_fwd8_k<64, true, 1>), g8, dim3(512), 0, st, a);
+            if (!a.causal && g_attn_opt[1]) hipLaunchKernelGGL((attn_fwd8_k<64, false, 1, 4, false>), g8, dim3(512), 0, st, a, NOQ);
+            else if (!a.causal && g_attn_opt[2]) hipLaunchKernelGGL((attn_fwd8_k<64, false, 1, 2, true>), g8, dim3(512), 0, st, a, NOQ);
+            else if (!a.causal) hipLaunchKernelGGL((attn_fwd8_k<64, false, 1>), g8, dim3(512), 0, st, a, NOQ);
+            else if (hpb == 2) hipLaunchKernelGGL((attn_fwd8_k<64, true, 2>), g8, dim3(512), 0, st, a, NOQ);
+            else hipLaunchKernelGGL((attn_fwd8_k<64, true, 1>), g8, dim3(512), 0, st, a, NOQ);
         }
         DESTA_CHECK_LAUNCH("attention_fwd");
         return DESTA_OK;
@@ -2167,11 +2374,16 @@
         const int hpb = !a.causal ? 1 : (d->head_dim == 128 ? (G % 4 == 0 ? 4 : (G % 2 == 0 ? 2 : 1)) : (G % 2 == 0 ? 2 : 1));
         const int rb = 256 / hpb;
         dim3 g8((unsigned)((a.Sq + rb - 1) / rb) * (unsigned)(G / hpb) * (unsigned)(a.B * a.Hkv));
+        int* const NOQ = nullptr;
         if (d->head_dim == 128) {
-            if (!a.causal) hipLaunchKernelGGL((attn_bwd_dq8_k<128, false, 1>), g8, dim3(512), 0, st, a, workspace);
-            else if (hpb == 4) hipLaunchKernelGGL((attn_bwd_dq8_k<128, true, 4>), g8, dim3(512), 0, st, a, workspace);
-            else if (hpb == 2) hipLaunchKernelGGL((attn_bwd_dq8_k<128, true, 2>), g8, dim3(512), 0, st, a, workspace);
-            else hipLaunchKernelGGL((attn_bwd_dq8_k<128, true, 1>), g8, dim3(512), 0, st, a, workspace);
+            if (!a.causal) hipLaunchKernelGGL((attn_bwd_dq8_k<128, false, 1>), g8, dim3(512), 0, st, a, workspace, NOQ);
+            else {
+#define DQ8_LAUNCH(HPB_) hipLaunchKernelGGL((attn_bwd_dq8_k<128, true, HPB_>), g8, dim3(512), 0, st, a, workspace, NOQ)
+                if (hpb == 4) DQ8_LAUNCH(4);
+                else if (hpb == 2) DQ8_LAUNCH(2);
+                else DQ8_LAUNCH(1);
+#undef DQ8_LAUNCH
+            }
             if (d->dK) {
                 if (g_attn_opt[5] && a.causal) {
                     dim3 gk2((unsigned)((a.Sk + 63) / 64) * a.Hkv * a.B);
@@ -2179,9 +2391,9 @@
                 } else hipLaunchKernelGGL((attn_bwd_dkdv_k<128, false>), gk_, dim3(256), 0, st, a);
             }
         } else {
-            if (!a.causal) hipLaunchKernelGGL((attn_bwd_dq8_k<64, false, 1>), g8, dim3(512), 0, st, a, workspace);
-            else if (hpb == 2) hipLaunchKernelGGL((attn_bwd_dq8_k<64, true, 2>), g8, dim3(512), 0, st, a, workspace);
-            else hipLaunchKernelGGL((attn_bwd_dq8_k<64, true, 1>), g8, dim3(512), 0, st, a, workspace);
+            if (!a.causal) hipLaunchKernelGGL((attn_bwd_dq8_k<64, false, 1>), g8, dim3(512), 0, st, a, workspace, NOQ);
+            else if (hpb == 2) hipLaunchKernelGGL((attn_bwd_dq8_k<64, true, 2>), g8, dim3(512), 0, st, a, workspace, NOQ);
+            else hipLaunchKernelGGL((attn_bwd_dq8_k<64, true, 1>), g8, dim3(512), 0, st, a, workspace, NOQ);
             if (d->dK) hipLaunchKernelGGL((attn_bwd_dkdv_k<64, false>), gk_, dim3(256), 0, st, a);
         }
         DESTA_CHECK_LAUNCH("attention_bwd");
diff --git a/desta2.5-audio_amd/desta/_hip.py b/desta2.5-audio_amd/desta/_hip.py
--- a/desta2.5-audio_amd/desta/_hip.py
+++ b/desta2.5-audio_amd/desta/_hip.py
@@ -745,6 +745,10 @@
         self.close()
 
 
+ATTN_OPT_PERSISTENT = 6
+ATTN_OPT_PERSISTENT_GRID = 7
+
+
 def attention_set_option(which: int, value: int) -> None:
     lib.desta_attention_set_option.argtypes = [i32, i32]
     check(lib.desta_attention_set_option(int(which), int(value)), "desta_attention_set_option")
```

Measured after the change: 6.486 (median of 2 runs). No clear change (+0.0%).
